# Geo3DSmart/PDANet

Hardware: AMD Instinct MI355X
Metric: scenes/sec (16384-pt ONCE, PDA-SSD forward+backward) (higher is better)
Workload: dtype f32; 1 GPU; once16k_b2_detector_fwd_bwd_adam; scenes_per_gpu=2, global_batch=2, parallelism=dp1, world_size_seen=1, cpu_affinity=GPU-local NUMA node of 0000:26:00.0: 128 CPUs, full=False, graph_tail=False, graph_head=True

## Files before the change

include/pda_train.h:

```cpp
#ifndef PDA_TRAIN_H
#define PDA_TRAIN_H
#include "pda_pointnet2.h"

#ifdef __cplusplus
extern "C" {
#endif

int pda_grad_norm(const float *g, int64_t n, float *norm_out, float *scratch1024, pda_stream_t stream);
int pda_adam_onecycle_step(float *p, const float *g, float *m, float *v, int64_t n, float lr,
                           float beta1, float beta2, float eps, float wd, int step,
                           const float *total_norm, float max_norm, pda_stream_t stream);

int64_t pda_bn_relu_scratch_bytes(int c);
int pda_bn_relu_fwd(const float *x, const float *gamma, const float *beta, float *running_mean,
                    float *running_var, float *y, float *mean_invstd, void *scratch, int64_t rows, int c,
                    float eps, float momentum, pda_stream_t stream);
int pda_bn_relu_bwd(const float *x, const float *grad_y, const float *gamma, const float *beta,
                    const float *mean_invstd, float *grad_x, float *grad_gamma, float *grad_beta,
                    void *scratch, int64_t rows, int c, pda_stream_t stream);
int pda_bn_relu_fwd_mixed(const void *x, int x_is_bf16, const float *gamma, const float *beta, float *running_mean,
                          float *running_var, void *y, int y_is_bf16, float *mean_invstd, void *scratch,
                          int64_t rows, int c, float eps, float momentum, pda_stream_t stream);
int pda_bn_relu_bwd_mixed(const void *x, int x_is_bf16, const void *grad_y, int grad_y_is_bf16, const float *gamma,
                          const float *beta, const float *mean_invstd, void *grad_x, float *grad_gamma,
                          float *grad_beta, void *scratch, int64_t rows, int c, pda_stream_t stream);
int pda_bn_relu_max_pool_fwd(const void *x, int x_is_bf16, const float *gamma, const float *beta, float *running_mean,
                             float *running_var, float *out, uint8_t *arg, float *mean_invstd, void *scratch,
                             int64_t groups, int ns, int c, float eps, float momentum, pda_stream_t stream);
int pda_bn_relu_max_pool_bwd(const void *x, int x_is_bf16, const float *grad_out, const uint8_t *arg,
                             const float *gamma, const float *beta, const float *mean_invstd, void *grad_x,
                             float *grad_gamma, float *grad_beta, void *scratch, int64_t groups, int ns, int c,
                             pda_stream_t stream);

int64_t pda_layer_norm_scratch_bytes(int d);
int pda_layer_norm_fwd(const float *x, const float *residual, const float *gamma, const float *beta,
                       float *sum_out, float *y, float *mean_rstd, int64_t rows, int d, float eps,
                       pda_stream_t stream);
int pda_layer_norm_bwd(const float *x, const float *grad_y, const float *grad_y2, const float *gamma,
                       const float *mean_rstd, float *grad_x, float *grad_gamma, float *grad_beta,
                       void *scratch, int64_t rows, int d, pda_stream_t stream);
int pda_layer_norm_fwd_mixed(const void *x, int x_is_bf16, const float *residual, const float *gamma,
                             const float *beta, float *sum_out, float *y, uint16_t *y_bf16, float *mean_rstd,
                             int64_t rows, int d, float eps, pda_stream_t stream);
int pda_layer_norm_bwd_mixed(const float *x, const float *grad_y, const void *grad_y2, int grad_y2_is_bf16,
                             const float *gamma, const float *mean_rstd, float *grad_x, uint16_t *grad_x_bf16,
                             float *grad_gamma, float *grad_beta, void *scratch, int64_t rows, int d,
                             pda_stream_t stream);

int64_t pda_linear_wgrad_scratch_bytes(int64_t tokens, int in_features, int out_features);
int pda_linear_wgrad_form(int64_t tokens, int in_features, int out_features);
int pda_linear_wgrad(const float *x, const float *grad_out, float *grad_weight, float *grad_bias,
                     void *scratch, int64_t tokens, int in_features, int out_features, pda_stream_t stream);
int pda_linear_wgrad_bn(const float *x, const float *grad_out, float *grad_weight, float *grad_bias, void *scratch,
                        int64_t tokens, int in_features, int out_features, const float *x_mean_invstd,
                        const float *x_gamma, const float *x_beta, pda_stream_t stream);

int64_t pda_gemm_split_bn_tiles(int64_t tokens);
int pda_gemm_split_bn(const float *x, const void *wf, float *y, int64_t tokens, int k, int n_out,
                      const float *in_mean_invstd, const float *in_gamma, const float *in_beta, int stats_mode,
                      double *partial, pda_stream_t stream);
int pda_gemm_split_maxpool(const float *x, const void *wf, const float *bias, float *out, int64_t tokens, int k, int n_out,
                           int ns, int relu, pda_stream_t stream);
int pda_gemm_split_gather(const float *point_rows, const float *xyz, const float *new_xyz, const int32_t *idx,
                          const float *w1, int ldw1, const float *bias1, const void *wf, const float *bias2, float *y,
                          int b, int n, int m, int ns, int k, int n_out, int relu, pda_stream_t stream);
int pda_bn_stats_fwd(const float *x, float *running_mean, float *running_var, float *mean_invstd, void *scratch,
                     int64_t rows, int c, float eps, float momentum, pda_stream_t stream);
int pda_bn_finalize_fwd(const double *partial, int nblocks, int c, int64_t count, float eps, float momentum,
                        float *mean_invstd, float *running_mean, float *running_var, pda_stream_t stream);
int pda_bn_relu_max_pool_apply(const float *x, const float *gamma, const float *beta, const float *mean_invstd,
                               float *out, uint8_t *arg, int64_t groups, int ns, int c, pda_stream_t stream);

int64_t pda_colsum_scratch_bytes(int cols);
int pda_colsum_bf16(const uint16_t *g, float *out, void *scratch, int64_t rows, int cols, pda_stream_t stream);

int pda_assemble_tokens(const float *rppe, const float *dscale, const float *feats, const int32_t *idx,
                        const float *glob, float *out, int b, int n, int m, int nsample, int c,
                        pda_stream_t stream);
int pda_assemble_tokens_grad(const float *grad_out, const float *dscale, const float *feats, const int32_t *idx,
                             float *grad_rppe, float *grad_dscale, float *grad_feats, float *grad_glob,
                             int b, int n, int m, int nsample, int c, pda_stream_t stream);

int pda_add_max_pool(const float *a, const float *b, float *out, uint8_t *arg, int64_t groups, int seq, int d,
                     pda_stream_t stream);
int pda_max_pool_scatter(const float *grad_out, const uint8_t *arg, float *grad_x, int64_t groups, int seq,
                         int d, pda_stream_t stream);
int pda_add_max_pool_bf16(const float *a, const uint16_t *b, float *out, uint8_t *arg, int64_t groups, int seq,
                          int d, pda_stream_t stream);
int pda_max_pool_scatter_bf16(const float *grad_out, const uint8_t *arg, float *grad_x, uint16_t *grad_x_bf16,
                              int64_t groups, int seq, int d, pda_stream_t stream);

int pda_bn_relu_fwd_weighted(const float *x, const float *gamma, const float *beta, float *running_mean,
                             float *running_var, float *y, float *mean_invstd, void *scratch, int64_t rows, int c,
                             float eps, float momentum, const float *row_weight, int64_t count, pda_stream_t stream);
int pda_bn_relu_bwd_weighted(const float *x, const float *grad_y, const float *gamma, const float *beta,
                             const float *mean_invstd, float *grad_x, float *grad_gamma, float *grad_beta,
                             void *scratch, int64_t rows, int c, const float *row_weight, int64_t count,
                             pda_stream_t stream);

int pda_ragged_plan(const int32_t *idx, int32_t *cnt, int32_t *off, int32_t *rowmap, float *row_weight, int64_t groups,
                    int nsample, pda_stream_t stream);
int pda_assemble_tokens_ragged(const float *rppe, const float *dscale, const float *feats, const int32_t *idx,
                               const float *glob, const int32_t *rowmap, const int32_t *off, float *out,
                               int64_t max_tokens, int b, int n, int m, int nsample, int c, int rppe_compact,
                               pda_stream_t stream);
int pda_assemble_tokens_ragged_grad(const float *grad_out, const float *dscale, const float *feats,
                                    const int32_t *idx, const int32_t *cnt, const int32_t *off, const int32_t *rowmap,
                                    float *grad_rppe, float *grad_dscale, float *grad_feats, float *grad_glob,
                                    int64_t max_tokens, int b, int n, int m, int nsample, int c, int rppe_compact,
                                    pda_stream_t stream);
int pda_add_max_pool_ragged(const float *a, const float *b, const int32_t *cnt, const int32_t *off, float *out,
                            uint8_t *arg, int64_t groups, int d, pda_stream_t stream);
int pda_max_pool_scatter_ragged(const float *grad_out, const uint8_t *arg, const int32_t *rowmap,
                                const int32_t *off, float *grad_x, int64_t max_tokens, int64_t groups, int nsample,
                                int d, pda_stream_t stream);
int pda_group_attention_ragged_fwd(const float *qkv, const int32_t *cnt, const int32_t *off, float *out, float *lse,
                                   int64_t tokens, int64_t num_groups, int seq, int heads, int head_dim,
                                   pda_stream_t stream);
int pda_group_attention_ragged_bwd(const float *qkv, const float *grad_out, const float *lse, const int32_t *cnt,
                                   const int32_t *off, float *grad_qkv, int64_t tokens, int64_t num_groups, int seq,
                                   int heads, int head_dim, pda_stream_t stream);

int pda_densitynet_param_count(void);
int64_t pda_densitynet_scratch_bytes(void);
int pda_densitynet_fwd(const float *x, const float *params, float *y, float *stats, void *scratch,
                       float *running_mean1, float *running_var1, float *running_mean2, float *running_var2,
                       float *running_mean3, float *running_var3, int64_t n, float eps, float momentum,
                       pda_stream_t stream);
int pda_densitynet_bwd(const float *x, const float *grad_y, const float *params, const float *stats,
                       float *grad_params, void *scratch, int64_t n, float eps, pda_stream_t stream);
int pda_densitynet_fwd_unique(const float *x, const float *params, float *y, float *stats, void *scratch,
                              float *running_mean1, float *running_var1, float *running_mean2, float *running_var2,
                              float *running_mean3, float *running_var3, int64_t n, const int32_t *rowmap,
                              const float *row_weight, const int32_t *n_unique, int nsample, float eps, float momentum,
                              pda_stream_t stream);
int pda_densitynet_bwd_unique(const float *x, const float *grad_y, const float *params, const float *stats,
                              float *grad_params, void *scratch, int64_t n, const int32_t *rowmap,
                              const float *row_weight, const int32_t *n_unique, int nsample, float eps,
                              pda_stream_t stream);
#define PDA_DENSITYNET_MAX_SCALES 4
typedef struct pda_densitynet_scale {
    const float *x, *grad_y, *params;
    float *y, *stats;
    void *scratch;
    float *running[6];
    float *grad_params;
    int64_t n;
    const int32_t *rowmap;
    const float *row_weight;
    const int32_t *n_unique;
    int nsample;
    float eps, momentum;
} pda_densitynet_scale_t;
int pda_densitynet_fwd_multi(const pda_densitynet_scale_t *scales, int nscales, pda_stream_t stream);
int pda_densitynet_bwd_multi(const pda_densitynet_scale_t *scales, int nscales, pda_stream_t stream);

int pda_densitynet_eval_param_count(void);
int pda_densitynet_eval(const float *x, const float *folded, float *y, int64_t n, pda_stream_t stream);

int pda_pda_geometry(const float *xyz, const float *new_xyz, const int32_t *idx, float *rppe, float *dscale,
                     int b, int n, int m, int nsample, float radius, pda_stream_t stream);

int pda_points_in_boxes(const float *boxes, const float *pts, int32_t *box_idx_of_points, int b, int t,
                        int m, pda_stream_t stream);
int pda_roiaware_pool3d_fwd(const float *rois, const float *pts, const float *pts_feature, int32_t *argmax,
                            int32_t *pts_idx_of_voxels, float *pooled_features, int boxes_num, int pts_num,
                            int channels, int max_pts_each_voxel, int out_x, int out_y, int out_z, int pool_method,
                            pda_stream_t stream);
int pda_roiaware_pool3d_bwd(const int32_t *pts_idx_of_voxels, const int32_t *argmax, const float *grad_out,
                            float *grad_in, int boxes_num, int pts_num, int channels, int max_pts_each_voxel,
                            int out_x, int out_y, int out_z, int pool_method, pda_stream_t stream);
int pda_roipoint_pool3d_fwd(const float *xyz, const float *boxes3d, const float *pts_feature, float *pooled_features,
                            int32_t *pooled_empty_flag, int batch_size, int pts_num, int boxes_num, int channels,
                            int sampled_pts_num, pda_stream_t stream);
int pda_points_in_boxes_mask(const float *boxes, const float *pts, int32_t *mask, int boxes_num, int pts_num,
                             pda_stream_t stream);
int pda_points_in_boxes_count(const float *points, int stride, const float *boxes, int32_t *counts, int pts_num,
                              int batch_size, int boxes_num, pda_stream_t stream);
int pda_assign_point_targets(const float *gt_boxes, const int32_t *in_box, const int32_t *in_ext, int64_t *labels,
                             int64_t *box_idx, float *gt_of_points, int b, int n, int t, int mode, int single_class,
                             pda_stream_t stream);
int pda_head_assign_targets(const float *points, int point_stride, int point_offset, const float *gt_boxes, const float *extra_width,
                            int64_t *labels, int64_t *box_idx, float *gt_of_points, float *box_labels, const float *mean_size,
                            int bins, int b, int n, int t, int mode, int single_class, pda_stream_t stream);
int pda_sa_gaussian_mask(const float *coords, int stride, int offset, const float *gt_of_points, const int64_t *labels,
                         float *out, int64_t points, pda_stream_t stream);

int pda_boxes_overlap_bev(const float *boxes_a, const float *boxes_b, float *ans_overlap, int num_a,
                          int num_b, pda_stream_t stream);
int pda_boxes_iou_bev(const float *boxes_a, const float *boxes_b, float *ans_iou, int num_a, int num_b,
                      pda_stream_t stream);
int64_t pda_nms_mask_words(int n);
int pda_nms_bev(const float *boxes, const int32_t *num_valid, int64_t *keep, int32_t *num_keep,
                uint64_t *mask_scratch, int b, int n, float thresh, int normal, pda_stream_t stream);

int pda_head_cls_loss(const float *preds, int row_stride, int col0, int num_class, const int64_t *labels, const float *soft,
                      int64_t n, float scale, float *out2, float *grad, pda_stream_t stream);
int pda_head_centerness(const float *centers, const float *gt, const int64_t *labels, float *out, int64_t n, pda_stream_t stream);
int pda_head_box_loss(const float *preds, const float *labels, const int64_t *cls_labels, const float *code_weights, float beta,
                      int bins, float dir_weight, float box_weight, int64_t n, float *out4, float *grad, pda_stream_t stream);
int pda_head_vote_loss(int mode, const float *origin, const float *offsets, const int64_t *key, const float *gt, int b, int boxes,
                       int num_class, float weight, int64_t n, float *out1, float *grad, pda_stream_t stream);
int pda_head_corner_loss(const float *box_preds, const float *centers, const float *cls_preds, int num_class, const float *gt,
                         const int64_t *cls_labels, const float *mean_size, int bins, float weight, int64_t n, float *out1,
                         float *grad_box, float *grad_centers, pda_stream_t stream);

int64_t pda_sa_small_train_workspace_bytes(void);
int pda_sa_small_train_supported(int c, int nsample, int c1, int c2, int c3, int64_t tokens);
int pda_sa_small_train_fwd(const float *xyz, const float *new_xyz, const float *feat_pm, const int32_t *idx,
                           const float *w1, const float *w2, const float *w3, const float *const *gamma,
                           const float *const *beta, float *const *running_mean, float *const *running_var,
                           const float *eps, const float *momentum, void *workspace, float *out, float *zmax,
                           uint8_t *arg, int b, int n, int m, int c, int nsample, int c1, int c2, int c3,
                           pda_stream_t stream);
int pda_sa_small_train_bwd(const float *xyz, const float *new_xyz, const float *feat_pm, const int32_t *idx,
                           const float *grad_out, const float *zmax, const uint8_t *arg, void *workspace, float *dz2,
                           float *dz1, float *dw1, float *dw2, float *dw3, float *const *dgamma, float *const *dbeta,
                           int b, int n, int m, int c, int nsample, int c1, int c2, int c3, pda_stream_t stream);

int64_t pda_sa_xyz_grad_scratch_bytes(int c1);
int pda_sa_point_gather(const float *point_rows, const float *xyz, const float *new_xyz, const int32_t *idx, const float *w,
                        int ldw, const float *bias, int relu, float *z, int b, int n, int m, int nsample, int c1,
                        pda_stream_t stream);
int pda_sa_xyz_grad(const float *grad_z1, const float *xyz, const float *new_xyz, const int32_t *idx, const float *w, int ldw,
                    float *dw, int lddw, float *grad_new_xyz, void *scratch, int b, int n, int m, int nsample, int c1,
                    pda_stream_t stream);

int64_t pda_input_stage_workspace_bytes(int batch, int64_t n_cap);
int pda_input_stage(const float *points, const int64_t *offsets, int64_t n_total, int batch, int c, int64_t n_cap,
                    const float *range6, int num_points, const int32_t *pick, const int32_t *perm1, const int32_t *perm2,
                    uint64_t seed, int shuffle, float *out_points, int32_t *info, void *workspace, pda_stream_t stream);
int pda_input_boxes(const float *boxes, const int64_t *box_offsets, int64_t m_total, int batch, int box_dim, int max_gt,
                    const float *range6, int min_num_corners, float *gt_boxes, int32_t *info, pda_stream_t stream);

int64_t pda_augment_workspace_bytes(int batch, int64_t n_cap, int k);
int pda_augment(const float *points, const int64_t *offsets, int64_t n_total, int batch, int c, int64_t n_cap,
                const float *boxes, const int64_t *box_offsets, int64_t m_total, const float *db_points,
                const int64_t *db_offsets, int64_t db_n_points, const float *db_boxes, const double *db_centre,
                const int32_t *db_class, int n_obj, const int32_t *cand, const int32_t *cand_group, const double *cand_dz,
                int k, const int32_t *flip, const double *angle, const float *scale, const float *remove_extra_width,
                int64_t paste_cap, float *out_points, int64_t out_cap, int64_t *out_offsets, float *out_boxes,
                int64_t out_box_cap, int64_t *out_box_offsets, int32_t *info, void *workspace, pda_stream_t stream);

int pda_augment_paste(const float *points, const int64_t *offsets, int64_t n_total, int batch, int c, int64_t n_cap,
                      const float *boxes, const int64_t *box_offsets, int64_t m_total, const float *db_points,
                      const int64_t *db_offsets, int64_t db_n_points, const float *db_boxes, const double *db_centre,
                      const int32_t *db_class, int n_obj, const int32_t *cand, const int32_t *cand_group,
                      const double *cand_dz, int k, const float *remove_extra_width, int64_t paste_cap, float *out_points,
                      int64_t out_cap, int64_t *out_offsets, float *out_boxes, int64_t out_box_cap,
                      int64_t *out_box_offsets, int32_t *info, void *workspace, pda_stream_t stream);

int64_t pda_augment_steps_workspace_bytes(int batch, int64_t n_cap, int box_slots, int n_ops);
int pda_augment_steps(const float *points, const int64_t *offsets, int64_t n_total, int batch, int c, int64_t n_cap,
                      const float *boxes, const int64_t *box_offsets, int64_t m_total, const int32_t *ops, int n_ops,
                      const double *scene_draws, const double *box_draws, int draw_cap, int box_slots,
                      const int32_t *info_in, float *out_points, int64_t out_cap, int64_t *out_offsets, float *out_boxes,
                      int64_t out_box_cap, int64_t *out_box_offsets, int32_t *info, void *workspace, pda_stream_t stream);

typedef struct pda_once_frames {
    const double *gt_boxes;
    const int32_t *gt_name;
    const int64_t *gt_offsets;
    const float *pred_boxes, *pred_score;
    const int32_t *pred_name;
    const int64_t *pred_start;
    const int32_t *pred_count;
    const int64_t *iou_start;
    int64_t n_gt_total, pred_cap, iou_cap;
    int n_frames, max_gt, max_pred;
} pda_once_frames_t;

int64_t pda_once_eval_workspace_bytes(int n_frames, int64_t n_gt_total, int n_tasks);
int pda_once_eval_iou(const pda_once_frames_t *frames, int with_heading, double *iou, int32_t *status,
                      pda_stream_t stream);
int pda_once_eval_accumulate(const pda_once_frames_t *frames, const double *iou, const uint8_t *accept, int n_classes,
                             int n_names, const double *iou_thr, int difficulty_mode, int64_t *num_valid_gt,
                             int32_t *status, void *workspace, pda_stream_t stream);
int pda_once_eval_match(const pda_once_frames_t *frames, const double *iou, const uint8_t *accept, int n_classes,
                        int n_names, const double *iou_thr, int difficulty_mode, int num_pr_points,
                        const float *sorted_scores, const int64_t *num_valid_gt, double *thresholds,
                        int64_t *n_thresholds, int64_t *counts, int32_t *status, void *workspace, pda_stream_t stream);


typedef struct pda_kitti_frames {
    const float *gt_bbox, *gt_loc;
    const double *gt_dims, *gt_ry, *gt_alpha, *gt_trunc, *gt_occ;
    const int32_t *gt_name;
    const int64_t *gt_offsets;
    const float *dt_bbox, *dt_box, *dt_alpha, *dt_score;
    const int32_t *dt_name;
    const int64_t *dt_start;
    const int32_t *dt_count;
    const int64_t *ov_start;
    const int32_t *frame_mode;
    int64_t n_gt_total, det_cap, ov_cap;
    int n_frames, max_gt, max_det;
} pda_kitti_frames_t;

int64_t pda_kitti_eval_workspace_bytes(int n_frames, int64_t n_gt_total, int64_t det_cap, int n_classes);
int pda_kitti_eval_overlaps(const pda_kitti_frames_t *frames, double *overlaps, int32_t *status, pda_stream_t stream);
int pda_kitti_eval_first_pass(const pda_kitti_frames_t *frames, const double *overlaps, int n_classes, int n_names,
                              const int8_t *gt_class, const uint8_t *dt_class, const uint8_t *dontcare,
                              const double *min_overlaps, int8_t *gt_flags, int8_t *dt_flags, int64_t *num_valid_gt,
                              int32_t *status, void *workspace, pda_stream_t stream);
int pda_kitti_eval_match(const pda_kitti_frames_t *frames, const double *overlaps, int n_classes, int n_names,
                         const int8_t *gt_class, const uint8_t *dt_class, const uint8_t *dontcare,
                         const double *min_overlaps, int compute_aos, const int8_t *gt_flags, const int8_t *dt_flags,
                         const float *sorted_scores, const int64_t *num_valid_gt, double *thresholds,
                         int64_t *n_thresholds, int64_t *counts, double *similarity, int32_t *status, void *workspace,
                         pda_stream_t stream);
int pda_kitti_eval_predictions(const float *boxes, int64_t n, int stride, int rows_per_frame, const int32_t *frame_idx,
                               const float *calib, const int32_t *image_shape, int n_frames, float *cam, float *bbox,
                               float *alpha, int32_t *status, pda_stream_t stream);

int pda_recall_record(const float *pred_boxes, const int32_t *num_pred, const float *gt_boxes, int gt_cols,
                      const float *thresh, int n_thresh, int64_t *counters, float *max_iou, int b, int k, int t,
                      pda_stream_t stream);

int pda_roi_max_iou(const float *rois, const int64_t *roi_labels, const float *gt_boxes, int gt_cols, int by_class,
                    float *max_overlaps, int32_t *gt_assignment, int b, int m, int t, pda_stream_t stream);
int pda_roi_sample_targets(const float *rois, const float *roi_scores, const int64_t *roi_labels, const float *gt_boxes,
                           int gt_cols, const float *max_overlaps, const int32_t *gt_assignment, int roi_per_image,
                           int fg_per_image, double hard_bg_ratio, double reg_fg_thresh, double cls_fg_thresh,
                           double cls_bg_thresh, double cls_bg_thresh_lo, int score_type, const int32_t *perm,
                           const double *fg_rand, const int64_t *hard_draw, const int64_t *easy_draw, uint64_t seed,
                           float *out_rois, float *gt_of_rois_src, float *gt_of_rois, float *gt_iou_of_rois,
                           float *out_roi_scores, int64_t *out_roi_labels, int64_t *reg_valid_mask, void *rcnn_cls_labels,
                           int32_t *sampled_inds, int32_t *status, int b, int m, int t, pda_stream_t stream);

int64_t pda_kitti_fov_filter_workspace_bytes(int batch, int64_t n_cap);
int pda_kitti_fov_filter(const float *points, const int64_t *offsets, int64_t n_total, int batch, int c, int64_t n_cap,
                         const float *calib, const int32_t *image_shape, float *out_points, int64_t out_cap,
                         int64_t *out_offsets, int32_t *info, void *workspace, pda_stream_t stream);
int64_t pda_gt_extract_workspace_bytes(int batch, int64_t n_cap, int64_t m_total);
int pda_gt_extract_count(const float *points, const int64_t *offsets, int64_t n_total, int batch, int c, int64_t n_cap,
                         const float *boxes, const int64_t *box_offsets, int64_t m_total, int32_t *counts, int32_t *info,
                         void *workspace, pda_stream_t stream);
int pda_gt_extract_write(const float *points, const int64_t *offsets, int64_t n_total, int batch, int c, int64_t n_cap,
                         const float *boxes, const int64_t *box_offsets, int64_t m_total, const double *centre,
                         const int64_t *obj_offsets, float *obj_points, int64_t out_cap, int32_t *info, void *workspace,
                         pda_stream_t stream);

int64_t pda_voxel_workspace_bytes(int batch, int64_t n_cap, int max_voxels, int max_points);
int pda_voxelize(const float *points, const int64_t *offsets, int64_t n_total, int batch, int c, int64_t n_cap,
                 const float *range6, const float *voxel_size3, const int32_t *grid3, int max_voxels, int max_points,
                 float *voxels, int32_t *coords, int32_t *num_points_per_voxel, int32_t *num_voxels, void *workspace,
                 pda_stream_t stream);
int pda_voxel_sample(const float *points, const int64_t *offsets, int64_t n_total, int batch, int c, int64_t n_cap,
                     const float *range6, const float *voxel_size3, const int32_t *grid3, int mask_xy, int max_voxels,
                     int max_points, int mean_vfe, int shuffle, const int32_t *perm0, const int64_t *perm0_offsets,
                     int64_t perm0_total, uint64_t seed, float *out_points, int64_t out_cap, int64_t *out_offsets,
                     int32_t *info, void *workspace, pda_stream_t stream);

int64_t pda_dyn_voxel_workspace_bytes(int64_t n, int key_bits);
int pda_dyn_voxel_index(const float *points, int64_t n, int columns, const float *range6, const float *voxel_size3,
                        const int32_t *grid3, int batch, int pillars, int32_t *counts, int32_t *point_idx, int32_t *unq_inv,
                        int32_t *unq_cnt, int32_t *voxel_coords, int32_t *seg_start, int32_t *seg_points, void *workspace,
                        pda_stream_t stream);
int pda_dyn_scatter_mean(const float *src, int columns, const int32_t *seg_start, const int32_t *seg_points,
                         const int32_t *counts, int64_t rows, float *out, pda_stream_t stream);
int pda_dyn_scatter_max_fwd(const float *x, int columns, const int32_t *seg_start, const int32_t *seg_points,
                            const int32_t *counts, int64_t rows, float *out, int32_t *arg, pda_stream_t stream);
int pda_dyn_scatter_max_bwd(const float *grad_out, const int32_t *arg, const int32_t *unq_inv, const int32_t *counts,
                            int64_t rows, int64_t vox_rows, int columns, float *grad_x, pda_stream_t stream);
int pda_dyn_pillar_features(const float *points, int64_t n, int columns, const int32_t *point_idx, const int32_t *unq_inv,
                            const int32_t *voxel_coords, const float *mean, const int32_t *counts, const float *voxel_size3,
                            const float *offset3, int absolute_xyz, int with_distance, float *out, pda_stream_t stream);

int pda_pillar_scatter_fwd(const float *features, const int32_t *coords, const int32_t *count, int64_t n, int c, int b, int ny,
                           int nx, float *out, pda_stream_t stream);
int pda_pillar_scatter_bwd(const float *grad_out, const int32_t *coords, const int32_t *count, int64_t n, int c, int b, int ny,
                           int nx, float *grad_features, pda_stream_t stream);
int pda_center_assign_targets(const float *gt_boxes, int gt_cols, int b, int m, int num_class, int n_heads,
                              const int32_t *head_of_class, const int32_t *local_of_class, const int32_t *head_classes, int h,
                              int w, int max_objs, double pcr0, double pcr1, double vs0, double vs1, double stride,
                              double gaussian_overlap, int min_radius, void *const *heatmaps, void *const *target_boxes,
                              void *const *inds, void *const *masks, pda_stream_t stream);
int64_t pda_center_focal_blocks(int64_t n);
int pda_center_focal_loss(const float *logits, const float *heatmap, int64_t n, float *grad, double *partials, float *out,
// ... 86 lines not shown
```

pdanet_amd/_lib.py:

```python
import ctypes
import os

_HERE = os.path.dirname(os.path.abspath(__file__))
LIB_PATH = os.environ.get("PDA_LIB_PATH") or os.path.join(_HERE, "libpda_pointnet2.so")
ABI_VERSION = 20


class DensityNetScale(ctypes.Structure):
    _fields_ = [("x", ctypes.c_void_p), ("grad_y", ctypes.c_void_p), ("params", ctypes.c_void_p), ("y", ctypes.c_void_p),
                ("stats", ctypes.c_void_p), ("scratch", ctypes.c_void_p), ("running", ctypes.c_void_p * 6),
                ("grad_params", ctypes.c_void_p), ("n", ctypes.c_int64), ("rowmap", ctypes.c_void_p),
                ("row_weight", ctypes.c_void_p), ("n_unique", ctypes.c_void_p), ("nsample", ctypes.c_int),
                ("eps", ctypes.c_float), ("momentum", ctypes.c_float)]


class OnceFrames(ctypes.Structure):
    _fields_ = [("gt_boxes", ctypes.c_void_p), ("gt_name", ctypes.c_void_p), ("gt_offsets", ctypes.c_void_p),
                ("pred_boxes", ctypes.c_void_p), ("pred_score", ctypes.c_void_p), ("pred_name", ctypes.c_void_p),
                ("pred_start", ctypes.c_void_p), ("pred_count", ctypes.c_void_p), ("iou_start", ctypes.c_void_p),
                ("n_gt_total", ctypes.c_int64), ("pred_cap", ctypes.c_int64), ("iou_cap", ctypes.c_int64),
                ("n_frames", ctypes.c_int), ("max_gt", ctypes.c_int), ("max_pred", ctypes.c_int)]


class KittiFrames(ctypes.Structure):
    _fields_ = [(n, ctypes.c_void_p) for n in ("gt_bbox", "gt_loc", "gt_dims", "gt_ry", "gt_alpha", "gt_trunc", "gt_occ",
                                               "gt_name", "gt_offsets", "dt_bbox", "dt_box", "dt_alpha", "dt_score",
                                               "dt_name", "dt_start", "dt_count", "ov_start", "frame_mode")] + \
               [("n_gt_total", ctypes.c_int64), ("det_cap", ctypes.c_int64), ("ov_cap", ctypes.c_int64),
                ("n_frames", ctypes.c_int), ("max_gt", ctypes.c_int), ("max_det", ctypes.c_int)]


PARAM_EPOCH = [0]
WEIGHT_EPOCH = [0]

_vp = ctypes.c_void_p
_i = ctypes.c_int
_f = ctypes.c_float

SIGNATURES = {
    "pda_furthest_point_sampling": [_vp, _vp, _vp, _i, _i, _i, _vp],
    "pda_furthest_point_sampling_with_dist": [_vp, _vp, _vp, _i, _i, _i, _vp],
    "pda_gather_points": [_vp, _vp, _vp, _i, _i, _i, _i, _vp],
    "pda_gather_points_grad": [_vp, _vp, _vp, _i, _i, _i, _i, _vp],
    "pda_ball_query": [_vp, _vp, _vp, _i, _i, _i, _f, _i, _vp],
    "pda_ball_query_dilated": [_vp, _vp, _vp, _i, _i, _i, _f, _f, _i, _vp],
    "pda_ellipsoid_query": [_vp, _vp, _vp, _i, _i, _i, _f, _f, _f, _i, _vp],
    "pda_ball_query_cells_scratch_bytes": [_i, _i],
    "pda_ball_query_cells": [_vp, _vp, ctypes.POINTER(_vp), _i, _i, _i, _i, ctypes.POINTER(_f), ctypes.POINTER(ctypes.c_int32),
                             _vp, ctypes.c_int64, _vp],
    "pda_ball_query_multi": [_vp, _vp, ctypes.POINTER(_vp), _i, _i, _i, _i,
                             ctypes.POINTER(_f), ctypes.POINTER(ctypes.c_int32), _vp],
    "pda_group_points": [_vp, _vp, _vp, _i, _i, _i, _i, _i, _vp],
    "pda_group_points_grad": [_vp, _vp, _vp, _i, _i, _i, _i, _i, _vp],
    "pda_group_rows": [_vp, _vp, _vp, _i, _i, _i, ctypes.c_int64, _vp],
    "pda_group_rows_grad": [_vp, _vp, _vp, _i, _i, _i, ctypes.c_int64, _vp],
    "pda_three_nn": [_vp, _vp, _vp, _vp, _i, _i, _i, _vp],
    "pda_three_interpolate": [_vp, _vp, _vp, _vp, _i, _i, _i, _i, _vp],
    "pda_three_interpolate_grad": [_vp, _vp, _vp, _vp, _i, _i, _i, _i, _vp],
    "pda_chamfer_forward": [_vp, _vp, _vp, _vp, _vp, _vp, _i, _i, _i, _vp],
    "pda_chamfer_backward": [_vp, _vp, _vp, _vp, _vp, _vp, _vp, _vp, _i, _i, _i, _vp],
    "pda_group_attention_fwd": [_vp, _vp, _vp, ctypes.c_int64, _i, _i, _i, _vp],
    "pda_group_attention_bwd": [_vp, _vp, _vp, _vp, ctypes.c_int64, _i, _i, _i, _vp],
    "pda_group_attention_fwd_bf16": [_vp, _vp, _vp, ctypes.c_int64, _i, _i, _i, _vp],
    "pda_group_attention_bwd_bf16": [_vp, _vp, _vp, _vp, ctypes.c_int64, _i, _i, _i, _vp],
    "pda_sa_mlp_maxpool": [_vp, _vp, _vp, _vp, _vp, _i, _i, _i, _i, _i, ctypes.POINTER(ctypes.c_int32),
                           ctypes.POINTER(_vp), ctypes.POINTER(_vp), ctypes.POINTER(_vp), _vp],
    "pda_linear_cols_packed_size": [_i, _i],
    "pda_linear_cols_pack": [_vp, _vp, _i, _i, _i, _i, _vp],
    "pda_linear_cols": [_vp, _vp, _vp, ctypes.c_int64, _i, _i, _vp],
    "pda_sa_gather_linear": [_vp, _vp, _vp, _vp, _vp, _vp, _i, _i, _i, _i, _i, _i, _vp],
    "pda_linear_split_packed_bytes": [_i, _i],
    "pda_linear_split_pack": [_vp, _vp, _i, _i, _i, _vp],
    "pda_linear_split_pack_both": [_vp, _vp, _vp, _i, _i, _vp],
    "pda_linear_split": [_vp, _vp, _vp, _vp, ctypes.c_int64, _i, _i, _i, _vp],
    "pda_gemm_split": [_vp, _vp, _vp, _vp, ctypes.c_int64, _i, _i, _i, _i, _vp],
    "pda_sa_mlp_packed_size": [_i, _i, _i],
    "pda_sa_mlp_pack_weights": [_vp, _vp, _i, _i, _i, _vp],
    "pda_grad_norm": [_vp, ctypes.c_int64, _vp, _vp, _vp],
    "pda_bn_relu_scratch_bytes": [_i],
    "pda_bn_relu_fwd": [_vp, _vp, _vp, _vp, _vp, _vp, _vp, _vp, ctypes.c_int64, _i, _f, _f, _vp],
    "pda_bn_relu_bwd": [_vp, _vp, _vp, _vp, _vp, _vp, _vp, _vp, _vp, ctypes.c_int64, _i, _vp],    "pda_bn_relu_fwd_mixed": [_vp, _i, _vp, _vp, _vp, _vp, _vp, _i, _vp, _vp, ctypes.c_int64, _i, _f, _f, _vp],
    "pda_bn_relu_bwd_mixed": [_vp, _i, _vp, _i, _vp, _vp, _vp, _vp, _vp, _vp, _vp, ctypes.c_int64, _i, _vp],
    "pda_bn_relu_max_pool_fwd": [_vp, _i, _vp, _vp, _vp, _vp, _vp, _vp, _vp, _vp, ctypes.c_int64, _i, _i, _f, _f, _vp],
    "pda_bn_relu_max_pool_bwd": [_vp, _i, _vp, _vp, _vp, _vp, _vp, _vp, _vp, _vp, _vp, ctypes.c_int64, _i, _i, _vp],

    "pda_layer_norm_scratch_bytes": [_i],
    "pda_layer_norm_fwd": [_vp, _vp, _vp, _vp, _vp, _vp, _vp, ctypes.c_int64, _i, _f, _vp],
    "pda_layer_norm_bwd": [_vp, _vp, _vp, _vp, _vp, _vp, _vp, _vp, _vp, ctypes.c_int64, _i, _vp],
    "pda_layer_norm_fwd_mixed": [_vp, _i, _vp, _vp, _vp, _vp, _vp, _vp, _vp, ctypes.c_int64, _i, _f, _vp],
    "pda_layer_norm_bwd_mixed": [_vp, _vp, _vp, _i, _vp, _vp, _vp, _vp, _vp, _vp, _vp, ctypes.c_int64, _i, _vp],
    "pda_linear_wgrad_scratch_bytes": [ctypes.c_int64, _i, _i],
    "pda_linear_wgrad_form": [ctypes.c_int64, _i, _i],
    "pda_linear_wgrad": [_vp, _vp, _vp, _vp, _vp, ctypes.c_int64, _i, _i, _vp],
    "pda_linear_wgrad_bn": [_vp, _vp, _vp, _vp, _vp, ctypes.c_int64, _i, _i, _vp, _vp, _vp, _vp],
    "pda_gemm_split_bn_tiles": [ctypes.c_int64],
    "pda_gemm_split_bn": [_vp, _vp, _vp, ctypes.c_int64, _i, _i, _vp, _vp, _vp, _i, _vp, _vp],
    "pda_gemm_split_maxpool": [_vp, _vp, _vp, _vp, ctypes.c_int64, _i, _i, _i, _i, _vp],
    "pda_gemm_split_gather": [_vp, _vp, _vp, _vp, _vp, _i, _vp, _vp, _vp, _vp, _i, _i, _i, _i, _i, _i, _i, _vp],
    "pda_bn_stats_fwd": [_vp, _vp, _vp, _vp, _vp, ctypes.c_int64, _i, _f, _f, _vp],
    "pda_bn_finalize_fwd": [_vp, _i, _i, ctypes.c_int64, _f, _f, _vp, _vp, _vp, _vp],
    "pda_bn_relu_max_pool_apply": [_vp, _vp, _vp, _vp, _vp, _vp, ctypes.c_int64, _i, _i, _vp],
    "pda_colsum_scratch_bytes": [_i],
    "pda_colsum_bf16": [_vp, _vp, _vp, ctypes.c_int64, _i, _vp],
    "pda_assemble_tokens": [_vp, _vp, _vp, _vp, _vp, _vp, _i, _i, _i, _i, _i, _vp],
    "pda_assemble_tokens_grad": [_vp, _vp, _vp, _vp, _vp, _vp, _vp, _vp, _i, _i, _i, _i, _i, _vp],
    "pda_add_max_pool": [_vp, _vp, _vp, _vp, ctypes.c_int64, _i, _i, _vp],
    "pda_max_pool_scatter": [_vp, _vp, _vp, ctypes.c_int64, _i, _i, _vp],
    "pda_add_max_pool_bf16": [_vp, _vp, _vp, _vp, ctypes.c_int64, _i, _i, _vp],
    "pda_max_pool_scatter_bf16": [_vp, _vp, _vp, _vp, ctypes.c_int64, _i, _i, _vp],
    "pda_ragged_plan": [_vp, _vp, _vp, _vp, _vp, ctypes.c_int64, _i, _vp],
    "pda_assemble_tokens_ragged": [_vp, _vp, _vp, _vp, _vp, _vp, _vp, _vp, ctypes.c_int64, _i, _i, _i, _i, _i, _i, _vp],
    "pda_assemble_tokens_ragged_grad": [_vp, _vp, _vp, _vp, _vp, _vp, _vp, _vp, _vp, _vp, _vp, ctypes.c_int64, _i, _i, _i, _i, _i, _i, _vp],
    "pda_bn_relu_fwd_weighted": [_vp, _vp, _vp, _vp, _vp, _vp, _vp, _vp, ctypes.c_int64, _i, _f, _f, _vp, ctypes.c_int64, _vp],
    "pda_bn_relu_bwd_weighted": [_vp, _vp, _vp, _vp, _vp, _vp, _vp, _vp, _vp, ctypes.c_int64, _i, _vp, ctypes.c_int64, _vp],
    "pda_add_max_pool_ragged": [_vp, _vp, _vp, _vp, _vp, _vp, ctypes.c_int64, _i, _vp],
    "pda_max_pool_scatter_ragged": [_vp, _vp, _vp, _vp, _vp, ctypes.c_int64, ctypes.c_int64, _i, _i, _vp],
    "pda_group_attention_ragged_fwd": [_vp, _vp, _vp, _vp, _vp, ctypes.c_int64, ctypes.c_int64, _i, _i, _i, _vp],
    "pda_group_attention_ragged_bwd": [_vp, _vp, _vp, _vp, _vp, _vp, ctypes.c_int64, ctypes.c_int64, _i, _i, _i, _vp],
    "pda_densitynet_param_count": [],
    "pda_densitynet_eval_param_count": [],
    "pda_densitynet_scratch_bytes": [],
    "pda_densitynet_fwd": [_vp, _vp, _vp, _vp, _vp, _vp, _vp, _vp, _vp, _vp, _vp, ctypes.c_int64, _f, _f, _vp],
    "pda_densitynet_bwd": [_vp, _vp, _vp, _vp, _vp, _vp, ctypes.c_int64, _f, _vp],
    "pda_densitynet_eval": [_vp, _vp, _vp, ctypes.c_int64, _vp],
    "pda_densitynet_fwd_multi": [_vp, _i, _vp],
    "pda_densitynet_bwd_multi": [_vp, _i, _vp],
    "pda_densitynet_fwd_unique": [_vp, _vp, _vp, _vp, _vp, _vp, _vp, _vp, _vp, _vp, _vp, ctypes.c_int64, _vp, _vp, _vp, _i, _f, _f, _vp],
    "pda_densitynet_bwd_unique": [_vp, _vp, _vp, _vp, _vp, _vp, ctypes.c_int64, _vp, _vp, _vp, _i, _f, _vp],
    "pda_pda_geometry": [_vp, _vp, _vp, _vp, _vp, _i, _i, _i, _i, _f, _vp],
    "pda_points_in_boxes": [_vp, _vp, _vp, _i, _i, _i, _vp],
    "pda_roiaware_pool3d_fwd": [_vp, _vp, _vp, _vp, _vp, _vp, _i, _i, _i, _i, _i, _i, _i, _i, _vp],
    "pda_roiaware_pool3d_bwd": [_vp, _vp, _vp, _vp, _i, _i, _i, _i, _i, _i, _i, _i, _vp],
    "pda_roipoint_pool3d_fwd": [_vp, _vp, _vp, _vp, _vp, _i, _i, _i, _i, _i, _vp],
    "pda_points_in_boxes_mask": [_vp, _vp, _vp, _i, _i, _vp],
    "pda_points_in_boxes_count": [_vp, _i, _vp, _vp, _i, _i, _i, _vp],
    "pda_assign_point_targets": [_vp, _vp, _vp, _vp, _vp, _vp, _i, _i, _i, _i, _i, _vp],
    "pda_sa_gaussian_mask": [_vp, _i, _i, _vp, _vp, _vp, ctypes.c_int64, _vp],
    "pda_head_assign_targets": [_vp, _i, _i, _vp, ctypes.POINTER(ctypes.c_float), _vp, _vp, _vp, _vp, _vp, _i, _i, _i, _i, _i, _i, _vp],
    "pda_head_cls_loss": [_vp, _i, _i, _i, _vp, _vp, ctypes.c_int64, _f, _vp, _vp, _vp],
    "pda_head_centerness": [_vp, _vp, _vp, _vp, ctypes.c_int64, _vp],
    "pda_head_box_loss": [_vp, _vp, _vp, _vp, _f, _i, _f, _f, ctypes.c_int64, _vp, _vp, _vp],
    "pda_head_vote_loss": [_i, _vp, _vp, _vp, _vp, _i, _i, _i, _f, ctypes.c_int64, _vp, _vp, _vp],
    "pda_head_corner_loss": [_vp, _vp, _vp, _i, _vp, _vp, _vp, _i, _f, ctypes.c_int64, _vp, _vp, _vp, _vp],
    "pda_boxes_overlap_bev": [_vp, _vp, _vp, _i, _i, _vp],
    "pda_boxes_iou_bev": [_vp, _vp, _vp, _i, _i, _vp],
    "pda_nms_mask_words": [_i],
    "pda_nms_bev": [_vp, _vp, _vp, _vp, _vp, _i, _i, _f, _i, _vp],
    "pda_sa_small_train_workspace_bytes": [],
    "pda_sa_small_train_supported": [_i, _i, _i, _i, _i, ctypes.c_int64],
    "pda_sa_small_train_fwd": [_vp] * 7 + [ctypes.POINTER(_vp)] * 4 + [ctypes.POINTER(_f)] * 2 + [_vp] * 4 + [_i] * 8 + [_vp],
    "pda_sa_small_train_bwd": [_vp] * 13 + [ctypes.POINTER(_vp)] * 2 + [_i] * 8 + [_vp],
    "pda_sa_xyz_grad_scratch_bytes": [_i],
    "pda_sa_point_gather": [_vp, _vp, _vp, _vp, _vp, _i, _vp, _i, _vp, _i, _i, _i, _i, _i, _vp],
    "pda_sa_xyz_grad": [_vp, _vp, _vp, _vp, _vp, _i, _vp, _i, _vp, _vp, _i, _i, _i, _i, _i, _vp],
    "pda_adam_onecycle_step": [_vp, _vp, _vp, _vp, ctypes.c_int64, _f, _f, _f, _f, _f, _i, _vp, _f, _vp],
    "pda_input_stage_workspace_bytes": [_i, ctypes.c_int64],
    "pda_input_stage": [_vp, _vp, ctypes.c_int64, _i, _i, ctypes.c_int64, ctypes.POINTER(_f), _i, _vp, _vp, _vp,
                        ctypes.c_uint64, _i, _vp, _vp, _vp, _vp],
    "pda_input_boxes": [_vp, _vp, ctypes.c_int64, _i, _i, _i, ctypes.POINTER(_f), _i, _vp, _vp, _vp],
    "pda_augment_workspace_bytes": [_i, ctypes.c_int64, _i],
    "pda_augment": [_vp, _vp, ctypes.c_int64, _i, _i, ctypes.c_int64, _vp, _vp, ctypes.c_int64, _vp, _vp, ctypes.c_int64, _vp,
                    _vp, _vp, _i, _vp, _vp, _vp, _i, _vp, _vp, _vp, ctypes.POINTER(_f), ctypes.c_int64, _vp, ctypes.c_int64,
                    _vp, _vp, ctypes.c_int64, _vp, _vp, _vp, _vp],
    "pda_augment_paste": [_vp, _vp, ctypes.c_int64, _i, _i, ctypes.c_int64, _vp, _vp, ctypes.c_int64, _vp, _vp, ctypes.c_int64, _vp,
                          _vp, _vp, _i, _vp, _vp, _vp, _i, ctypes.POINTER(_f), ctypes.c_int64, _vp, ctypes.c_int64, _vp, _vp,
                          ctypes.c_int64, _vp, _vp, _vp, _vp],
    "pda_augment_steps_workspace_bytes": [_i, ctypes.c_int64, _i, _i],
    "pda_augment_steps": [_vp, _vp, ctypes.c_int64, _i, _i, ctypes.c_int64, _vp, _vp, ctypes.c_int64,
                          ctypes.POINTER(ctypes.c_int32), _i, _vp, _vp, _i, _i, _vp, _vp, ctypes.c_int64, _vp, _vp,
                          ctypes.c_int64, _vp, _vp, _vp, _vp],
    "pda_once_eval_workspace_bytes": [_i, ctypes.c_int64, _i],
    "pda_once_eval_iou": [ctypes.POINTER(OnceFrames), _i, _vp, _vp, _vp],
    "pda_once_eval_accumulate": [ctypes.POINTER(OnceFrames), _vp, _vp, _i, _i, ctypes.POINTER(ctypes.c_double), _i, _vp, _vp,
                                 _vp, _vp],
    "pda_once_eval_match": [ctypes.POINTER(OnceFrames), _vp, _vp, _i, _i, ctypes.POINTER(ctypes.c_double), _i, _i, _vp, _vp,
                            _vp, _vp, _vp, _vp, _vp, _vp],
    "pda_kitti_eval_workspace_bytes": [_i, ctypes.c_int64, ctypes.c_int64, _i],
    "pda_kitti_eval_overlaps": [ctypes.POINTER(KittiFrames), _vp, _vp, _vp],
    "pda_kitti_eval_first_pass": [ctypes.POINTER(KittiFrames), _vp, _i, _i, _vp, _vp, _vp, ctypes.POINTER(ctypes.c_double),
                                  _vp, _vp, _vp, _vp, _vp, _vp],
    "pda_kitti_eval_match": [ctypes.POINTER(KittiFrames), _vp, _i, _i, _vp, _vp, _vp, ctypes.POINTER(ctypes.c_double), _i,
                             _vp, _vp, _vp, _vp, _vp, _vp, _vp, _vp, _vp, _vp, _vp],
    "pda_kitti_eval_predictions": [_vp, ctypes.c_int64, _i, _i, _vp, _vp, _vp, _i, _vp, _vp, _vp, _vp, _vp],
    "pda_recall_record": [_vp, _vp, _vp, _i, ctypes.POINTER(_f), _i, _vp, _vp, _i, _i, _i, _vp],
    "pda_roi_max_iou": [_vp, _vp, _vp, _i, _i, _vp, _vp, _i, _i, _i, _vp],
    "pda_roi_sample_targets": [_vp, _vp, _vp, _vp, _i, _vp, _vp, _i, _i] + [ctypes.c_double] * 5 + [_i, _vp, _vp, _vp, _vp,
                               ctypes.c_uint64] + [_vp] * 10 + [_i, _i, _i, _vp],
    "pda_kitti_fov_filter_workspace_bytes": [_i, ctypes.c_int64],
    "pda_kitti_fov_filter": [_vp, _vp, ctypes.c_int64, _i, _i, ctypes.c_int64, _vp, _vp, _vp, ctypes.c_int64, _vp, _vp, _vp, _vp],
    "pda_gt_extract_workspace_bytes": [_i, ctypes.c_int64, ctypes.c_int64],
    "pda_gt_extract_count": [_vp, _vp, ctypes.c_int64, _i, _i, ctypes.c_int64, _vp, _vp, ctypes.c_int64, _vp, _vp, _vp, _vp],
    "pda_gt_extract_write": [_vp, _vp, ctypes.c_int64, _i, _i, ctypes.c_int64, _vp, _vp, ctypes.c_int64, _vp, _vp, _vp,
                             ctypes.c_int64, _vp, _vp, _vp],
    "pda_voxel_workspace_bytes": [_i, ctypes.c_int64, _i, _i],
    "pda_voxelize": [_vp, _vp, ctypes.c_int64, _i, _i, ctypes.c_int64, ctypes.POINTER(_f), ctypes.POINTER(_f),
                     ctypes.POINTER(ctypes.c_int32), _i, _i, _vp, _vp, _vp, _vp, _vp, _vp],
    "pda_voxel_sample": [_vp, _vp, ctypes.c_int64, _i, _i, ctypes.c_int64, ctypes.POINTER(_f), ctypes.POINTER(_f),
                         ctypes.POINTER(ctypes.c_int32), _i, _i, _i, _i, _i, _vp, _vp, ctypes.c_int64, ctypes.c_uint64, _vp,
                         ctypes.c_int64, _vp, _vp, _vp, _vp],
    "pda_dyn_voxel_workspace_bytes": [ctypes.c_int64, _i],
    "pda_dyn_voxel_index": [_vp, ctypes.c_int64, _i, ctypes.POINTER(_f), ctypes.POINTER(_f), ctypes.POINTER(ctypes.c_int32),
                            _i, _i, _vp, _vp, _vp, _vp, _vp, _vp, _vp, _vp, _vp],
    "pda_dyn_scatter_mean": [_vp, _i, _vp, _vp, _vp, ctypes.c_int64, _vp, _vp],
    "pda_dyn_scatter_max_fwd": [_vp, _i, _vp, _vp, _vp, ctypes.c_int64, _vp, _vp, _vp],
    "pda_dyn_scatter_max_bwd": [_vp, _vp, _vp, _vp, ctypes.c_int64, ctypes.c_int64, _i, _vp, _vp],
    "pda_dyn_pillar_features": [_vp, ctypes.c_int64, _i, _vp, _vp, _vp, _vp, _vp, ctypes.POINTER(_f), ctypes.POINTER(_f), _i,
                                _i, _vp, _vp],
    "pda_pillar_scatter_fwd": [_vp, _vp, _vp, ctypes.c_int64, _i, _i, _i, _i, _vp, _vp],
    "pda_pillar_scatter_bwd": [_vp, _vp, _vp, ctypes.c_int64, _i, _i, _i, _i, _vp, _vp],
    "pda_center_assign_targets": [_vp, _i, _i, _i, _i, _i] + [ctypes.POINTER(ctypes.c_int32)] * 3 + [_i, _i, _i]
                                 + [ctypes.c_double] * 6 + [_i] + [ctypes.POINTER(_vp)] * 4 + [_vp],
    "pda_center_focal_blocks": [ctypes.c_int64],
    "pda_center_focal_loss": [_vp, _vp, ctypes.c_int64, _vp, _vp, _vp, _vp],
    "pda_center_scale": [_vp, _vp, _vp, _f, ctypes.c_int64, _vp, _vp],
    "pda_center_reg_loss": [ctypes.POINTER(_vp), ctypes.POINTER(ctypes.c_int32), _i, _vp, _vp, _vp, ctypes.POINTER(_f), _f, _i,
                            _i, ctypes.c_int64, _vp, _vp],
    "pda_center_reg_loss_grad": [ctypes.POINTER(_vp), ctypes.POINTER(ctypes.c_int32), _i, _vp, _vp, _vp, ctypes.POINTER(_f), _f,
                                 _i, _i, ctypes.c_int64, _vp, _vp, ctypes.POINTER(_vp), _vp],
    "pda_center_decode": [_vp] * 7 + [_i] * 5 + [ctypes.POINTER(ctypes.c_int32)] + [ctypes.c_double] * 5
                         + [ctypes.POINTER(_f), _i, ctypes.c_double, _vp, _vp, _vp, _vp],
    "pda_anchor_assign_targets": [_vp, _i, _i, _i, _vp, _i, _i, ctypes.POINTER(ctypes.c_int32), ctypes.POINTER(_f),
                                  ctypes.POINTER(_f), ctypes.POINTER(ctypes.c_int32), _vp, _vp, _vp, _vp, _vp, _vp],
    "pda_anchor_loss_blocks": [ctypes.c_int64],
    "pda_anchor_loss": [_vp] * 7 + [_i] * 4 + [ctypes.POINTER(_f)] + [ctypes.c_double] * 4 + [_vp] * 6,
    "pda_anchor_decode": [_vp, _vp, _vp, _i, _i, _i, ctypes.c_double, ctypes.c_double, _vp, _vp],
    "pda_pillar_features": [_vp, _vp, _vp, ctypes.c_int64, _i, _i, ctypes.POINTER(_f), ctypes.POINTER(_f), _i, _i, _vp, _vp],
    "pda_spconv_index_workspace_bytes": [ctypes.c_int64, ctypes.c_int64, _i],
    "pda_spconv_index_subm": [_vp, ctypes.c_int64] + [_i] * 7 + [_vp, _vp, _vp, _vp],
    "pda_spconv_index_strided": [_vp, ctypes.c_int64] + [_i] * 13 + [ctypes.c_int64, _vp, _vp, _vp, _vp, _vp, _vp],
    "pda_spconv_gemm": [_vp, _vp, _vp, _vp, _vp, ctypes.c_int64, ctypes.c_int64, _i, _i, _i, _i, _i, _vp],
    "pda_spconv_wgrad_workspace_bytes": [ctypes.c_int64, _i, _i, _i],
    "pda_spconv_wgrad": [_vp, _vp, _vp, ctypes.c_int64, ctypes.c_int64, _i, _i, _i, _vp, _vp, _vp, _vp],
    "pda_voxel_pool_scratch_doubles": [_i, _i, _i],
    "pda_voxel_pool_moments": [_vp, _vp, _vp, _vp, _vp, _i, _i, _i, _vp],
    "pda_voxel_pool_fwd": [_vp] * 9 + [_i, _i, _i, _i, _vp],
    "pda_voxel_pool_bwd": [_vp] * 10 + [_i, _i, _i, _i, _vp],
    "pda_stack_sa_scratch_doubles": [_i, _i, _i, _i],
    "pda_stack_sa_moments": [_vp] * 9 + [_i] * 5 + [_vp],
    "pda_stack_sa_fwd": [_vp] * 15 + [_i] * 6 + [_vp],
    "pda_stack_sa_apply": [_vp, _vp, _vp, _vp, _i, _i, _vp],
    "pda_stack_sa_bwd1": [_vp] * 18 + [_i] * 6 + [_vp],
    "pda_stack_sa_bwd2": [_vp] * 14 + [_i] * 5 + [_vp],
    "pda_bev_interpolate_fwd": [_vp] * 5 + [_i] * 5 + [_vp],
    "pda_bev_interpolate_bwd": [_vp] * 5 + [_i] * 5 + [_vp],
    "pda_bev_roi_grid_pool": [_vp] * 3 + [_i] * 6 + [_f] * 4 + [_vp],
    "pda_stack_ball_query": [_vp, _vp, _vp, _vp, _vp, _i, _i, _f, _i, _vp],
    "pda_stack_group_points": [_vp, _vp, _vp, _vp, _vp, _i, _i, _i, _i, _vp],
    "pda_stack_group_points_grad": [_vp, _vp, _vp, _vp, _vp, _i, _i, _i, _i, _i, _vp],
    "pda_stack_furthest_point_sampling": [_vp, _vp, _vp, _vp, _vp, _i, _vp],
    "pda_stack_three_nn": [_vp, _vp, _vp, _vp, _vp, _vp, _i, _i, _vp],
    "pda_stack_three_interpolate": [_vp, _vp, _vp, _vp, _i, _i, _vp],
    "pda_stack_three_interpolate_grad": [_vp, _vp, _vp, _vp, _i, _i, _vp],
    "pda_stack_voxel_query": [_vp, _vp, _vp, _vp, _vp, _i, _i, _i, _i, _i, _i, _i, _f, _i, _i, _i, _vp],
    "pda_stack_query_local_neighbor_idxs": [_vp, _vp, _vp, _vp, _vp, _vp, _vp, _i, _f, _i, _i, _i, _i, _vp],
    "pda_stack_three_nn_by_local_idxs": [_vp, _vp, _vp, _vp, _vp, _vp, _i, ctypes.c_int64, _i, _i, _vp],
    "pda_stack_vector_pool": [_vp, _vp, _vp, _vp, _vp, _vp, _vp, _vp, _vp, _vp, _i, _i, _i, _i, _i, _i, _i, _i, _f, _i, _i,
                              _i, _i, _i, _vp],
    "pda_stack_vector_pool_grad": [_vp, _vp, _vp, _vp, _i, _i, _i, _i, _i, _i, _vp],
}
SIZE_QUERIES = [
    "pda_nms_mask_words", "pda_ball_query_cells_scratch_bytes", "pda_bn_relu_scratch_bytes",
    "pda_layer_norm_scratch_bytes", "pda_linear_wgrad_scratch_bytes", "pda_linear_split_packed_bytes",
    "pda_colsum_scratch_bytes", "pda_gemm_split_bn_tiles", "pda_densitynet_scratch_bytes",
    "pda_sa_small_train_workspace_bytes", "pda_sa_xyz_grad_scratch_bytes", "pda_input_stage_workspace_bytes",
    "pda_augment_workspace_bytes", "pda_augment_steps_workspace_bytes", "pda_once_eval_workspace_bytes",
    "pda_kitti_eval_workspace_bytes", "pda_kitti_fov_filter_workspace_bytes", "pda_gt_extract_workspace_bytes",
    "pda_voxel_workspace_bytes", "pda_dyn_voxel_workspace_bytes", "pda_center_focal_blocks", "pda_anchor_loss_blocks",
    "pda_spconv_index_workspace_bytes", "pda_spconv_wgrad_workspace_bytes", "pda_voxel_pool_scratch_doubles",
    "pda_stack_sa_scratch_doubles"]
INFO_SYMBOLS = ["pda_abi_version", "pda_last_error", "pda_fp_contract_mode", "pda_opt_n_threads",
                "pda_fps_coop_timeouts", "pda_debug_fps_spin_limit", "pda_debug_fps_exchange_nonzero"]

_LIB = None


class PdaError(RuntimeError):
    pass


def load():
    global _LIB
    if _LIB is not None:
        return _LIB
    import torch
    if not os.path.exists(LIB_PATH):
        raise PdaError(
            "%s not found: build it with `python -m pdanet_amd.build` (hipcc, gfx950). "
            "pdanet_amd has no fallback path." % LIB_PATH)
    lib = ctypes.CDLL(LIB_PATH)
    for name, argtypes in SIGNATURES.items():
        fn = getattr(lib, name)
        fn.argtypes = argtypes
        fn.restype = _i
    for name in SIZE_QUERIES:
        getattr(lib, name).restype = ctypes.c_int64
    lib.pda_abi_version.restype = _i
    lib.pda_last_error.restype = ctypes.c_char_p
    lib.pda_fp_contract_mode.restype = _i
    lib.pda_opt_n_threads.argtypes = [_i]
    lib.pda_opt_n_threads.restype = _i
    lib.pda_fps_coop_timeouts.argtypes = [ctypes.POINTER(ctypes.c_ulonglong), _i]
    lib.pda_fps_coop_timeouts.restype = _i
    lib.pda_debug_fps_spin_limit.argtypes = [_i]
    lib.pda_debug_fps_spin_limit.restype = _i
    lib.pda_debug_fps_exchange_nonzero.argtypes = []
    lib.pda_debug_fps_exchange_nonzero.restype = ctypes.c_longlong
    if lib.pda_abi_version() != ABI_VERSION:
        raise PdaError("libpda_pointnet2.so ABI %d != binding ABI %d: rebuild"
                       % (lib.pda_abi_version(), ABI_VERSION))
    _LIB = lib
    return lib


def check(status, what):
    if status != 0:
        msg = load().pda_last_error().decode("utf-8", "replace")
        raise PdaError("%s failed with status %d: %s" % (what, status, msg))
```

pdanet_amd/csrc/bn_relu.hip:

```cpp
#include "pda_common.h"

namespace pda {

constexpr int BN_BLOCKS = 512;

struct BnShape {
    int64_t rows;
    int c, cg, rpb;
    int ns;
    const float* roww;
    int64_t count;
};

__device__ __forceinline__ float4 pooled_grad(const float* __restrict__ gout, const uint8_t* __restrict__ arg, int64_t r,
                                              int col, const BnShape& s) {
    const int64_t g = r / s.ns;
    const int t = (int)(r - g * s.ns);
    const float4 v = reinterpret_cast<const float4*>(gout)[g * s.cg + col];
    const uchar4 k = reinterpret_cast<const uchar4*>(arg)[g * s.cg + col];
    return make_float4(k.x == t ? v.x : 0.f, k.y == t ? v.y : 0.f, k.z == t ? v.z : 0.f, k.w == t ? v.w : 0.f);
}

__device__ __forceinline__ void block_reduce_cols(double (&a)[4], double (&b)[4], double* lds, int cg, int rpb, double* out_a,
                                                  double* out_b) {
// ... 175 lines not shown
}

template <typename TX>
__global__ __launch_bounds__(256) void bn_apply_pool_kernel(const TX* __restrict__ x, const float* __restrict__ mean_invstd,
                                                            const float* __restrict__ gamma, const float* __restrict__ beta,
                                                            float* __restrict__ out, uint8_t* __restrict__ arg, int64_t groups,
                                                            BnShape s) {
    const int64_t e = (int64_t)blockIdx.x * 256 + threadIdx.x;
    if (e >= groups * s.cg) return;
    const int64_t g = e / s.cg;
    const int col = (int)(e - g * s.cg);
    const float4 mu = reinterpret_cast<const float4*>(mean_invstd)[col], is = reinterpret_cast<const float4*>(mean_invstd + s.c)[col];
    const float4 gm = reinterpret_cast<const float4*>(gamma)[col], be = reinterpret_cast<const float4*>(beta)[col];
    float4 best = make_float4(-1.f, -1.f, -1.f, -1.f);
    uchar4 bi = make_uchar4(0, 0, 0, 0);
    const TX* px = x + (size_t)g * s.ns * s.c + 4 * col;
    for (int t = 0; t < s.ns; ++t) {
        const float4 v = load4(px + (size_t)t * s.c);
        const float y0 = fmaxf((v.x - mu.x) * is.x * gm.x + be.x, 0.f), y1 = fmaxf((v.y - mu.y) * is.y * gm.y + be.y, 0.f);
        const float y2 = fmaxf((v.z - mu.z) * is.z * gm.z + be.z, 0.f), y3 = fmaxf((v.w - mu.w) * is.w * gm.w + be.w, 0.f);
        if (y0 > best.x) { best.x = y0; bi.x = (uint8_t)t; }
        if (y1 > best.y) { best.y = y1; bi.y = (uint8_t)t; }
        if (y2 > best.z) { best.z = y2; bi.z = (uint8_t)t; }
        if (y3 > best.w) { best.w = y3; bi.w = (uint8_t)t; }
    }
    reinterpret_cast<float4*>(out)[e] = best;
    reinterpret_cast<uchar4*>(arg)[e] = bi;
}

static int bn_shape(int64_t rows, int c, BnShape& s, const char* what) {
    PDA_REQUIRE(rows >= 1, "%s: rows = %lld", what, (long long)rows);
    PDA_REQUIRE(c >= 4 && c <= 1024 && (c & (c - 1)) == 0, "%s: C = %d is not a power of two in [4, 1024]", what, c);
    s.rows = rows; s.c = c; s.cg = c / 4; s.rpb = 256 / s.cg; s.ns = 1;
    s.roww = nullptr; s.count = rows;
    return PDA_OK;
}

static int bn_grid(const BnShape& s) {
    const int64_t steps = divup64(s.rows, s.rpb);
    return (int)(steps < BN_BLOCKS ? steps : BN_BLOCKS);
}

}

PDA_API int64_t pda_bn_relu_scratch_bytes(int c) {
    const int64_t cc = c > 0 ? c : 0;
    return (int64_t)pda::BN_BLOCKS * 2 * cc * (int64_t)sizeof(double) + 2 * cc * (int64_t)sizeof(float);
}

namespace pda {

template <typename T> static bool bn_aligned(const T* p) { return ((uintptr_t)p & (4 * sizeof(T) - 1)) == 0; }

template <typename TX, typename TY>
static int launch_bn_relu_fwd(const TX* x, const float* gamma, const float* beta, float* running_mean, float* running_var, TY* y,
                              float* mean_invstd, void* scratch, int64_t rows, int c, float eps, float momentum, hipStream_t st,
                              const char* what, const float* roww = nullptr, int64_t count = 0) {
    BnShape s;
    if (int rc = bn_shape(rows, c, s, what)) return rc;
    if (roww) { PDA_REQUIRE(count >= rows, "%s: count = %lld < rows", what, (long long)count); s.roww = roww; s.count = count; }
    PDA_REQUIRE(x && gamma && beta && y && mean_invstd && scratch, "%s: null pointer", what);
    PDA_REQUIRE((running_mean == nullptr) == (running_var == nullptr), "%s: running_mean/var must come together", what);
    PDA_REQUIRE(bn_aligned(x) && bn_aligned(y) && (((uintptr_t)gamma | (uintptr_t)beta | (uintptr_t)mean_invstd) & 15) == 0,
                "%s: pointers must be 16-byte aligned (8 for bf16 tensors)", what);
    const int grid = bn_grid(s);
    hipLaunchKernelGGL((bn_reduce_kernel<false, TX, float>), dim3(grid), dim3(256), 0, st, x, (const float*)nullptr, (const float*)nullptr,
                       (const float*)nullptr, (const float*)nullptr, (double*)scratch, s);
    hipLaunchKernelGGL(bn_finalize_fwd_kernel, dim3(divup(c, 32)), dim3(512), 0, st, (const double*)scratch, grid, c, s.count, eps, momentum,
                       mean_invstd, running_mean, running_var);
    hipLaunchKernelGGL((bn_apply_kernel<false, TX, float, TY>), dim3(grid), dim3(256), 0, st, x, (const float*)nullptr, mean_invstd, gamma, beta,
                       (const float*)nullptr, y, s);
    return check_launch(what);
}

template <typename TX, typename TD>
static int launch_bn_relu_bwd(const TX* x, const TD* grad_y, const float* gamma, const float* beta, const float* mean_invstd, TX* grad_x,
                              float* grad_gamma, float* grad_beta, void* scratch, int64_t rows, int c, hipStream_t st, const char* what,
                              const float* roww = nullptr, int64_t count = 0) {
    BnShape s;
    if (int rc = bn_shape(rows, c, s, what)) return rc;
    if (roww) { PDA_REQUIRE(count >= rows, "%s: count = %lld < rows", what, (long long)count); s.roww = roww; s.count = count; }
    PDA_REQUIRE(x && grad_y && gamma && beta && mean_invstd && grad_x && grad_gamma && grad_beta && scratch, "%s: null pointer", what);
    PDA_REQUIRE(bn_aligned(x) && bn_aligned(grad_y) && bn_aligned(grad_x) && (((uintptr_t)gamma | (uintptr_t)beta | (uintptr_t)mean_invstd) & 15) == 0,
                "%s: pointers must be 16-byte aligned (8 for bf16 tensors)", what);
    const int grid = bn_grid(s);
    float* sums = reinterpret_cast<float*>(reinterpret_cast<double*>(scratch) + (size_t)BN_BLOCKS * 2 * c);
    hipLaunchKernelGGL((bn_reduce_kernel<true, TX, TD>), dim3(grid), dim3(256), 0, st, x, grad_y, mean_invstd, gamma, beta, (double*)scratch, s);
    hipLaunchKernelGGL(bn_finalize_bwd_kernel, dim3(divup(c, 32)), dim3(512), 0, st, (const double*)scratch, grid, c, s.count, grad_gamma, grad_beta,
                       sums);
    hipLaunchKernelGGL((bn_apply_kernel<true, TX, TD, TX>), dim3(grid), dim3(256), 0, st, x, grad_y, mean_invstd, gamma, beta, sums, grad_x, s);
    return check_launch(what);
}

template <typename TX>
static int launch_bn_relu_pool_fwd(const TX* x, const float* gamma, const float* beta, float* running_mean, float* running_var, float* out,
                                   uint8_t* arg, float* mean_invstd, void* scratch, int64_t groups, int ns, int c, float eps,
                                   float momentum, hipStream_t st, const char* what) {
    PDA_REQUIRE(groups >= 1 && ns >= 1 && ns <= 255, "%s: groups=%lld ns=%d (1..255)", what, (long long)groups, ns);
    BnShape s;
    if (int rc = bn_shape(groups * ns, c, s, what)) return rc;
    s.ns = ns;
    PDA_REQUIRE(x && gamma && beta && out && arg && mean_invstd && scratch, "%s: null pointer", what);
    PDA_REQUIRE((running_mean == nullptr) == (running_var == nullptr), "%s: running_mean/var must come together", what);
    PDA_REQUIRE(bn_aligned(x) && (((uintptr_t)out | (uintptr_t)gamma | (uintptr_t)beta | (uintptr_t)mean_invstd) & 15) == 0 &&
                    ((uintptr_t)arg & 3) == 0, "%s: alignment", what);
    const int grid = bn_grid(s);
    hipLaunchKernelGGL((bn_reduce_kernel<false, TX, float>), dim3(grid), dim3(256), 0, st, x, (const float*)nullptr, (const float*)nullptr,
                       (const float*)nullptr, (const float*)nullptr, (double*)scratch, s, (const uint8_t*)nullptr);
    hipLaunchKernelGGL(bn_finalize_fwd_kernel, dim3(divup(c, 32)), dim3(512), 0, st, (const double*)scratch, grid, c, s.rows, eps, momentum,
                       mean_invstd, running_mean, running_var);
    hipLaunchKernelGGL(bn_apply_pool_kernel<TX>, dim3((unsigned)divup64(groups * s.cg, 256)), dim3(256), 0, st, x, mean_invstd, gamma, beta, out,
                       arg, groups, s);
    return check_launch(what);
}

template <typename TX>
static int launch_bn_relu_pool_bwd(const TX* x, const float* grad_out, const uint8_t* arg, const float* gamma, const float* beta,
                                   const float* mean_invstd, TX* grad_x, float* grad_gamma, float* grad_beta, void* scratch, int64_t groups,
                                   int ns, int c, hipStream_t st, const char* what) {
    PDA_REQUIRE(groups >= 1 && ns >= 1 && ns <= 255, "%s: groups=%lld ns=%d (1..255)", what, (long long)groups, ns);
    BnShape s;
    if (int rc = bn_shape(groups * ns, c, s, what)) return rc;
    s.ns = ns;
    PDA_REQUIRE(x && grad_out && arg && gamma && beta && mean_invstd && grad_x && grad_gamma && grad_beta && scratch, "%s: null pointer", what);
    PDA_REQUIRE(bn_aligned(x) && bn_aligned(grad_x) && (((uintptr_t)grad_out | (uintptr_t)gamma | (uintptr_t)beta | (uintptr_t)mean_invstd) & 15) == 0 &&
                    ((uintptr_t)arg & 3) == 0, "%s: alignment", what);
    const int grid = bn_grid(s);
    float* sums = reinterpret_cast<float*>(reinterpret_cast<double*>(scratch) + (size_t)BN_BLOCKS * 2 * c);
    hipLaunchKernelGGL((bn_reduce_kernel<true, TX, float, true>), dim3(grid), dim3(256), 0, st, x, grad_out, mean_invstd, gamma, beta,
                       (double*)scratch, s, arg);
    hipLaunchKernelGGL(bn_finalize_bwd_kernel, dim3(divup(c, 32)), dim3(512), 0, st, (const double*)scratch, grid, c, s.rows, grad_gamma, grad_beta,
                       sums);
    hipLaunchKernelGGL((bn_apply_kernel<true, TX, float, TX, true>), dim3(grid), dim3(256), 0, st, x, grad_out, mean_invstd, gamma, beta, sums,
                       grad_x, s, arg);
    return check_launch(what);
}

}

PDA_API int pda_bn_relu_fwd(const float* x, const float* gamma, const float* beta, float* running_mean, float* running_var,
                            float* y, float* mean_invstd, void* scratch, int64_t rows, int c, float eps, float momentum,
                            pda_stream_t stream) {
    return pda::launch_bn_relu_fwd<float, float>(x, gamma, beta, running_mean, running_var, y, mean_invstd, scratch, rows, c, eps, momentum,
                                                 (hipStream_t)stream, "pda_bn_relu_fwd");
}

PDA_API int pda_bn_relu_bwd(const float* x, const float* grad_y, const float* gamma, const float* beta, const float* mean_invstd,
                            float* grad_x, float* grad_gamma, float* grad_beta, void* scratch, int64_t rows, int c,
                            pda_stream_t stream) {
    return pda::launch_bn_relu_bwd<float, float>(x, grad_y, gamma, beta, mean_invstd, grad_x, grad_gamma, grad_beta, scratch, rows, c,
                                                 (hipStream_t)stream, "pda_bn_relu_bwd");
}

PDA_API int pda_bn_relu_fwd_weighted(const float* x, const float* gamma, const float* beta, float* running_mean, float* running_var,
                                     float* y, float* mean_invstd, void* scratch, int64_t rows, int c, float eps, float momentum,
                                     const float* row_weight, int64_t count, pda_stream_t stream) {
    PDA_REQUIRE(row_weight != nullptr, "pda_bn_relu_fwd_weighted: null pointer");
    return pda::launch_bn_relu_fwd<float, float>(x, gamma, beta, running_mean, running_var, y, mean_invstd, scratch, rows, c, eps, momentum,
                                                 (hipStream_t)stream, "pda_bn_relu_fwd_weighted", row_weight, count);
}

PDA_API int pda_bn_relu_bwd_weighted(const float* x, const float* grad_y, const float* gamma, const float* beta, const float* mean_invstd,
                                     float* grad_x, float* grad_gamma, float* grad_beta, void* scratch, int64_t rows, int c,
                                     const float* row_weight, int64_t count, pda_stream_t stream) {
    PDA_REQUIRE(row_weight != nullptr, "pda_bn_relu_bwd_weighted: null pointer");
    return pda::launch_bn_relu_bwd<float, float>(x, grad_y, gamma, beta, mean_invstd, grad_x, grad_gamma, grad_beta, scratch, rows, c,
                                                 (hipStream_t)stream, "pda_bn_relu_bwd_weighted", row_weight, count);
}

PDA_API int pda_bn_relu_fwd_mixed(const void* x, int x_is_bf16, const float* gamma, const float* beta, float* running_mean,
                                  float* running_var, void* y, int y_is_bf16, float* mean_invstd, void* scratch, int64_t rows, int c,
                                  float eps, float momentum, pda_stream_t stream) {
    using pda::bf16_t;
    hipStream_t st = (hipStream_t)stream;
    const char* what = "pda_bn_relu_fwd_mixed";
#define PDA_BN_FWD(TX, TY) pda::launch_bn_relu_fwd<TX, TY>((const TX*)x, gamma, beta, running_mean, running_var, (TY*)y, mean_invstd, scratch, rows, c, eps, momentum, st, what)
    if (x_is_bf16) return y_is_bf16 ? PDA_BN_FWD(bf16_t, bf16_t) : PDA_BN_FWD(bf16_t, float);
    return y_is_bf16 ? PDA_BN_FWD(float, bf16_t) : PDA_BN_FWD(float, float);
#undef PDA_BN_FWD
}

PDA_API int pda_bn_relu_bwd_mixed(const void* x, int x_is_bf16, const void* grad_y, int grad_y_is_bf16, const float* gamma,
                                  const float* beta, const float* mean_invstd, void* grad_x, float* grad_gamma, float* grad_beta,
                                  void* scratch, int64_t rows, int c, pda_stream_t stream) {
    using pda::bf16_t;
    hipStream_t st = (hipStream_t)stream;
    const char* what = "pda_bn_relu_bwd_mixed";
#define PDA_BN_BWD(TX, TD) pda::launch_bn_relu_bwd<TX, TD>((const TX*)x, (const TD*)grad_y, gamma, beta, mean_invstd, (TX*)grad_x, grad_gamma, grad_beta, scratch, rows, c, st, what)
    if (x_is_bf16) return grad_y_is_bf16 ? PDA_BN_BWD(bf16_t, bf16_t) : PDA_BN_BWD(bf16_t, float);
    return grad_y_is_bf16 ? PDA_BN_BWD(float, bf16_t) : PDA_BN_BWD(float, float);
#undef PDA_BN_BWD
}

PDA_API int pda_bn_relu_max_pool_fwd(const void* x, int x_is_bf16, const float* gamma, const float* beta, float* running_mean,
                                     float* running_var, float* out, uint8_t* arg, float* mean_invstd, void* scratch, int64_t groups,
                                     int ns, int c, float eps, float momentum, pda_stream_t stream) {
    const char* what = "pda_bn_relu_max_pool_fwd";
    if (x_is_bf16)
        return pda::launch_bn_relu_pool_fwd<pda::bf16_t>((const pda::bf16_t*)x, gamma, beta, running_mean, running_var, out, arg, mean_invstd,
                                                         scratch, groups, ns, c, eps, momentum, (hipStream_t)stream, what);
    return pda::launch_bn_relu_pool_fwd<float>((const float*)x, gamma, beta, running_mean, running_var, out, arg, mean_invstd, scratch, groups,
                                               ns, c, eps, momentum, (hipStream_t)stream, what);
}

PDA_API int pda_bn_relu_max_pool_bwd(const void* x, int x_is_bf16, const float* grad_out, const uint8_t* arg, const float* gamma,
                                     const float* beta, const float* mean_invstd, void* grad_x, float* grad_gamma, float* grad_beta,
                                     void* scratch, int64_t groups, int ns, int c, pda_stream_t stream) {
    const char* what = "pda_bn_relu_max_pool_bwd";
    if (x_is_bf16)
        return pda::launch_bn_relu_pool_bwd<pda::bf16_t>((const pda::bf16_t*)x, grad_out, arg, gamma, beta, mean_invstd, (pda::bf16_t*)grad_x,
                                                         grad_gamma, grad_beta, scratch, groups, ns, c, (hipStream_t)stream, what);
    return pda::launch_bn_relu_pool_bwd<float>((const float*)x, grad_out, arg, gamma, beta, mean_invstd, (float*)grad_x, grad_gamma, grad_beta,
                                               scratch, groups, ns, c, (hipStream_t)stream, what);
}

PDA_API int pda_bn_stats_fwd(const float* x, float* running_mean, float* running_var, float* mean_invstd, void* scratch, int64_t rows, int c,
                             float eps, float momentum, pda_stream_t stream) {
    const char* what = "pda_bn_stats_fwd";
    pda::BnShape s;
    if (int rc = pda::bn_shape(rows, c, s, what)) return rc;
    PDA_REQUIRE(x && mean_invstd && scratch && pda::bn_aligned(x) && ((uintptr_t)mean_invstd & 15) == 0, "%s: null or misaligned pointer", what);
    PDA_REQUIRE((running_mean == nullptr) == (running_var == nullptr), "%s: running_mean/var must come together", what);
    const int grid = pda::bn_grid(s);
    hipStream_t st = (hipStream_t)stream;
    hipLaunchKernelGGL((pda::bn_reduce_kernel<false, float, float>), dim3(grid), dim3(256), 0, st, x, (const float*)nullptr, (const float*)nullptr,
                       (const float*)nullptr, (const float*)nullptr, (double*)scratch, s);
    hipLaunchKernelGGL(pda::bn_finalize_fwd_kernel, dim3(pda::divup(c, 32)), dim3(512), 0, st, (const double*)scratch, grid, c, s.count, eps, momentum,
                       mean_invstd, running_mean, running_var);
    return pda::check_launch(what);
}

PDA_API int pda_bn_finalize_fwd(const double* partial, int nblocks, int c, int64_t count, float eps, float momentum, float* mean_invstd,
                                float* running_mean, float* running_var, pda_stream_t stream) {
    PDA_REQUIRE(partial && mean_invstd && nblocks >= 1 && c >= 1 && count >= 1, "pda_bn_finalize_fwd: bad argument");
    PDA_REQUIRE((running_mean == nullptr) == (running_var == nullptr), "pda_bn_finalize_fwd: running_mean/var must come together");
    hipLaunchKernelGGL(pda::bn_finalize_fwd_kernel, dim3(pda::divup(c, 32)), dim3(512), 0, (hipStream_t)stream, partial, nblocks, c, count, eps,
                       momentum, mean_invstd, running_mean, running_var);
    return pda::check_launch("pda_bn_finalize_fwd");
}

PDA_API int pda_bn_relu_max_pool_apply(const float* x, const float* gamma, const float* beta, const float* mean_invstd, float* out, uint8_t* arg,
                                       int64_t groups, int ns, int c, pda_stream_t stream) {
    const char* what = "pda_bn_relu_max_pool_apply";
    PDA_REQUIRE(groups >= 1 && ns >= 1 && ns <= 255, "%s: groups=%lld ns=%d (1..255)", what, (long long)groups, ns);
    pda::BnShape s;
    if (int rc = pda::bn_shape(groups * ns, c, s, what)) return rc;
    s.ns = ns;
    PDA_REQUIRE(x && gamma && beta && out && arg && mean_invstd, "%s: null pointer", what);
    PDA_REQUIRE(pda::bn_aligned(x) && (((uintptr_t)out | (uintptr_t)gamma | (uintptr_t)beta | (uintptr_t)mean_invstd) & 15) == 0 &&
                    ((uintptr_t)arg & 3) == 0, "%s: alignment", what);
    hipLaunchKernelGGL(pda::bn_apply_pool_kernel<float>, dim3((unsigned)pda::divup64(groups * s.cg, 256)), dim3(256), 0, (hipStream_t)stream, x,
                       mean_invstd, gamma, beta, out, arg, groups, s);
    return pda::check_launch(what);
}
```

pdanet_amd/csrc/sa_xyz_grad.hip:

```cpp
#include "pda_common.h"

namespace pda {

constexpr int XG_BLOCKS = 512;
constexpr int XG_THREADS = 256;
constexpr int XG_MAXC = 4;

template <int CPT>
__global__ __launch_bounds__(XG_THREADS) void sa_xyz_grad_kernel(const float* __restrict__ g, const float* __restrict__ xyz,
                                                                 const float* __restrict__ new_xyz, const int32_t* __restrict__ idx,
                                                                 const float* __restrict__ w, int ldw, float* __restrict__ partial,
                                                                 float* __restrict__ grad_new, int n, int m, int ns, int c1, int64_t groups) {
    __shared__ float red[XG_THREADS / 64][3];
    const int tid = threadIdx.x;
    float accw[CPT][3], wx[CPT][3];
#pragma unroll
    for (int q = 0; q < CPT; ++q) {
        const int o = tid + q * XG_THREADS;
#pragma unroll
        for (int d = 0; d < 3; ++d) { accw[q][d] = 0.f; wx[q][d] = o < c1 ? w[(size_t)o * ldw + d] : 0.f; }
    }
    for (int64_t grp = blockIdx.x; grp < groups; grp += gridDim.x) {
        const int bs = (int)(grp / m);
        const float* ct = new_xyz + grp * 3;
        const float cx = ct[0], cy = ct[1], cz = ct[2];
        const float* pts = xyz + (size_t)bs * n * 3;
        const int32_t* ids = idx + grp * ns;
        const float* grow = g + grp * ns * (int64_t)c1;
        float gs[CPT];
#pragma unroll
        for (int q = 0; q < CPT; ++q) gs[q] = 0.f;
        for (int s0 = 0; s0 < ns; s0 += 8) {
            float gv[8][CPT], dx[8], dy[8], dz[8];
#pragma unroll
            for (int u = 0; u < 8; ++u) {
                const int s = s0 + u < ns ? s0 + u : ns - 1;
                const float* pt = pts + (size_t)ids[s] * 3;
                dx[u] = pt[0] - cx; dy[u] = pt[1] - cy; dz[u] = pt[2] - cz;
#pragma unroll
                for (int q = 0; q < CPT; ++q) {
                    const int o = tid + q * XG_THREADS;
                    gv[u][q] = (s0 + u < ns && o < c1) ? grow[(int64_t)s * c1 + o] : 0.f;
                }
            }
#pragma unroll
            for (int u = 0; u < 8; ++u)
#pragma unroll
                for (int q = 0; q < CPT; ++q) {
                    accw[q][0] = __builtin_fmaf(gv[u][q], dx[u], accw[q][0]);
                    accw[q][1] = __builtin_fmaf(gv[u][q], dy[u], accw[q][1]);
                    accw[q][2] = __builtin_fmaf(gv[u][q], dz[u], accw[q][2]);
                    gs[q] += gv[u][q];
                }
        }
        if (grad_new) {
            float v[3] = {0.f, 0.f, 0.f};
#pragma unroll
            for (int q = 0; q < CPT; ++q)
#pragma unroll
                for (int d = 0; d < 3; ++d) v[d] = __builtin_fmaf(gs[q], wx[q][d], v[d]);
#pragma unroll
            for (int d = 0; d < 3; ++d) {
#pragma unroll
                for (int o = 32; o >= 1; o >>= 1) v[d] += __shfl_xor(v[d], o);
            }
            __syncthreads();
            if (lane_id() == 0) { red[wave_id()][0] = v[0]; red[wave_id()][1] = v[1]; red[wave_id()][2] = v[2]; }
            __syncthreads();
            if (tid < 3) grad_new[grp * 3 + tid] = -((red[0][tid] + red[1][tid]) + (red[2][tid] + red[3][tid]));
        }
    }
#pragma unroll
    for (int q = 0; q < CPT; ++q) {
        const int o = tid + q * XG_THREADS;
        if (o < c1) {
            float* p = partial + ((size_t)blockIdx.x * c1 + o) * 3;
            p[0] = accw[q][0]; p[1] = accw[q][1]; p[2] = accw[q][2];
        }
    }
}

__global__ __launch_bounds__(256) void sa_xyz_grad_reduce_kernel(const float* __restrict__ partial, int nblocks, int c1, float* __restrict__ dw, int lddw) {
    __shared__ double red[16][16];
    const int el = threadIdx.x & 15, part = threadIdx.x >> 4;
    const int e = blockIdx.x * 16 + el;
    const bool ok = e < c1 * 3;
    double a = 0.0;
    if (ok)
        for (int k = part; k < nblocks; k += 16) a += (double)partial[(size_t)k * c1 * 3 + e];
    red[part][el] = a;
    __syncthreads();
    if (part == 0 && ok) {
        double t = 0.0;
#pragma unroll
        for (int q = 0; q < 16; ++q) t += red[q][el];
        dw[(size_t)(e / 3) * lddw + e % 3] = (float)t;
    }
}

__global__ __launch_bounds__(256) void sa_point_gather_kernel(const float* __restrict__ prow, const float* __restrict__ xyz,
                                                              const float* __restrict__ new_xyz, const int32_t* __restrict__ idx,
                                                              const float* __restrict__ w, int ldw, const float* __restrict__ bias,
                                                              int relu, float* __restrict__ z, int n, int m, int ns, int c1,
                                                              int64_t tokens) {
    const int cq = c1 >> 2;
    const int q = threadIdx.x % cq;
    float wx[4], wy[4], wz[4];
#pragma unroll
    for (int k = 0; k < 4; ++k) {
        const float* wr = w + (size_t)(4 * q + k) * ldw;
        wx[k] = wr[0]; wy[k] = wr[1]; wz[k] = wr[2];
    }
    float bq[4] = {0.f, 0.f, 0.f, 0.f};
    if (bias) { const float4 b4 = *reinterpret_cast<const float4*>(bias + 4 * q); bq[0] = b4.x; bq[1] = b4.y; bq[2] = b4.z; bq[3] = b4.w; }
    const int tpb = 256 / cq;
    for (int64_t tok = (int64_t)blockIdx.x * tpb + threadIdx.x / cq; tok < tokens; tok += (int64_t)gridDim.x * tpb) {
        const int64_t grp = tok / ns;
        const int bs = (int)(grp / m);
        const int id = idx[tok];
        const float* pt = xyz + ((size_t)bs * n + id) * 3;
        const float* ct = new_xyz + grp * 3;
        const float dx = pt[0] - ct[0], dy = pt[1] - ct[1], dz = pt[2] - ct[2];
        const float4 p4 = *reinterpret_cast<const float4*>(prow + ((size_t)bs * n + id) * c1 + 4 * q);
        const float pv[4] = {p4.x, p4.y, p4.z, p4.w};
        float o[4];
#pragma unroll
        for (int k = 0; k < 4; ++k) {
            o[k] = __builtin_fmaf(wz[k], dz, __builtin_fmaf(wy[k], dy, __builtin_fmaf(wx[k], dx, pv[k]))) + bq[k];
            o[k] = relu ? fmaxf(o[k], 0.f) : o[k];
        }
        *reinterpret_cast<float4*>(z + tok * c1 + 4 * q) = make_float4(o[0], o[1], o[2], o[3]);
    }
}

}

PDA_API int pda_sa_point_gather(const float* point_rows, const float* xyz, const float* new_xyz, const int32_t* idx, const float* w, int ldw,
                                const float* bias, int relu, float* z, int b, int n, int m, int ns, int c1, pda_stream_t stream) {
    using namespace pda;
    PDA_REQUIRE(b >= 0 && n >= 1 && m >= 0 && ns >= 1 && c1 >= 4 && (c1 & 3) == 0 && ldw >= 3, "pda_sa_point_gather: bad size");
    const int64_t tokens = (int64_t)b * m * ns;
    if (tokens == 0) return PDA_OK;
    PDA_REQUIRE(point_rows && xyz && new_xyz && idx && w && z && (((uintptr_t)point_rows | (uintptr_t)z | (uintptr_t)bias) & 15) == 0,
                "pda_sa_point_gather: null or misaligned pointer");
    if (256 % (c1 >> 2) != 0) {
        set_error("pda_sa_point_gather: c1 = %d (c1 / 4 must divide 256)", c1);
        return PDA_ERR_UNSUPPORTED;
    }
    const int64_t total = tokens * (c1 >> 2);
    const int blocks = (int)(divup64(total, 256) < 8192 ? divup64(total, 256) : 8192);
    hipLaunchKernelGGL(sa_point_gather_kernel, dim3(blocks), dim3(256), 0, (hipStream_t)stream, point_rows, xyz, new_xyz, idx, w, ldw, bias, relu, z,
                       n, m, ns, c1, tokens);
    return check_launch("pda_sa_point_gather");
}

PDA_API int64_t pda_sa_xyz_grad_scratch_bytes(int c1) { return c1 > 0 ? (int64_t)pda::XG_BLOCKS * c1 * 3 * sizeof(float) : 0; }

PDA_API int pda_sa_xyz_grad(const float* grad_z1, const float* xyz, const float* new_xyz, const int32_t* idx, const float* w, int ldw,
                            float* dw, int lddw, float* grad_new_xyz, void* scratch, int b, int n, int m, int ns, int c1,
                            pda_stream_t stream) {
    using namespace pda;
    PDA_REQUIRE(b >= 0 && n >= 1 && m >= 0 && ns >= 1 && c1 >= 1 && ldw >= 3 && lddw >= 3, "pda_sa_xyz_grad: bad size");
    const int64_t groups = (int64_t)b * m;
    if (groups == 0) return PDA_OK;
    PDA_REQUIRE(grad_z1 && xyz && new_xyz && idx && w && dw && scratch, "pda_sa_xyz_grad: null pointer");
    if (c1 > XG_THREADS * XG_MAXC) {
        set_error("pda_sa_xyz_grad: c1 = %d > %d", c1, XG_THREADS * XG_MAXC);
        return PDA_ERR_UNSUPPORTED;
    }
    const hipStream_t s = (hipStream_t)stream;
    const int blocks = (int)(groups < XG_BLOCKS ? groups : XG_BLOCKS);
    float* partial = (float*)scratch;
    const int cpt = divup(c1, XG_THREADS);
#define PDA_XG(CPT) hipLaunchKernelGGL((sa_xyz_grad_kernel<CPT>), dim3(blocks), dim3(XG_THREADS), 0, s, grad_z1, xyz, new_xyz, idx, w, ldw, \
                                       partial, grad_new_xyz, n, m, ns, c1, groups)
    if (cpt == 1) PDA_XG(1); else if (cpt == 2) PDA_XG(2); else PDA_XG(4);
#undef PDA_XG
    hipLaunchKernelGGL(sa_xyz_grad_reduce_kernel, dim3(divup(c1 * 3, 16)), dim3(256), 0, s, (const float*)partial, blocks, c1, dw, lddw);
    return check_launch("pda_sa_xyz_grad");
}
```

pdanet_amd/pointnet2_batch_cuda.py:

```python
import ctypes

import functools

import torch

from . import _lib
from . import param_cache


def _chk(t, name, dtype):
    if not isinstance(t, torch.Tensor):
        raise TypeError("%s must be a torch.Tensor" % name)
    if not t.is_cuda:
        raise RuntimeError("%s must be a CUDA(HIP) tensor -- there is no CPU path" % name)
    if not t.is_contiguous():
        raise RuntimeError("%s must be contiguous" % name)
    if t.dtype != dtype:
        raise RuntimeError("%s must be %s, got %s" % (name, dtype, t.dtype))
    return t.data_ptr()


def _numel_ok(t, n, name):
    if t.numel() < n:
        raise RuntimeError("%s has %d elements, the sizes passed need %d" % (name, t.numel(), n))
# ... 113 lines not shown
    _numel_ok(idx, b * npoints * nsample, "idx"); _numel_ok(grad_points, b * c * n, "grad_points")
    _call("pda_group_points_grad", grad_out, _chk(grad_out, "grad_out", F32), _chk(idx, "idx", I32),
          _chk(grad_points, "grad_points", F32), b, c, n, npoints, nsample)
    return 1


def group_rows(b, n, c, num_idx, rows, idx, out):
    _numel_ok(rows, b * n * c, "rows"); _numel_ok(idx, b * num_idx, "idx"); _numel_ok(out, b * num_idx * c, "out")
    _call("pda_group_rows", rows, _chk(rows, "rows", F32), _chk(idx, "idx", I32), _chk(out, "out", F32),
          b, n, c, num_idx)
    return 1


def group_rows_grad(b, n, c, num_idx, grad_out, idx, grad_rows):
    _numel_ok(grad_out, b * num_idx * c, "grad_out"); _numel_ok(idx, b * num_idx, "idx")
    _numel_ok(grad_rows, b * n * c, "grad_rows")
    _call("pda_group_rows_grad", grad_out, _chk(grad_out, "grad_out", F32), _chk(idx, "idx", I32),
          _chk(grad_rows, "grad_rows", F32), b, n, c, num_idx)
    return 1


def gather_points_wrapper(b, c, n, npoints, points, idx, out):
    _numel_ok(points, b * c * n, "points"); _numel_ok(idx, b * npoints, "idx")
    _numel_ok(out, b * c * npoints, "out")
    _call("pda_gather_points", points, _chk(points, "points", F32), _chk(idx, "idx", I32),
          _chk(out, "out", F32), b, c, n, npoints)
    return 1


def gather_points_grad_wrapper(b, c, n, npoints, grad_out, idx, grad_points):
    _numel_ok(grad_out, b * c * npoints, "grad_out"); _numel_ok(idx, b * npoints, "idx")
    _numel_ok(grad_points, b * c * n, "grad_points")
    _call("pda_gather_points_grad", grad_out, _chk(grad_out, "grad_out", F32), _chk(idx, "idx", I32),
          _chk(grad_points, "grad_points", F32), b, c, n, npoints)
    return 1


def farthest_point_sampling_wrapper(b, n, m, xyz, temp, idx):
    _numel_ok(xyz, b * n * 3, "xyz"); _numel_ok(temp, b * n, "temp"); _numel_ok(idx, b * m, "idx")
    _call("pda_furthest_point_sampling", xyz, _chk(xyz, "xyz", F32), _chk(temp, "temp", F32),
          _chk(idx, "idx", I32), b, n, m)
    return 1


def furthest_point_sampling_with_dist_wrapper(b, n, m, dist, temp, idx):
    _numel_ok(dist, b * n * n, "dist"); _numel_ok(temp, b * n, "temp"); _numel_ok(idx, b * m, "idx")
    _call("pda_furthest_point_sampling_with_dist", dist, _chk(dist, "dist", F32),
          _chk(temp, "temp", F32), _chk(idx, "idx", I32), b, n, m)
    return 2


def three_nn_wrapper(b, n, m, unknown, known, dist2, idx):
    _numel_ok(unknown, b * n * 3, "unknown"); _numel_ok(known, b * m * 3, "known")
    _numel_ok(dist2, b * n * 3, "dist2"); _numel_ok(idx, b * n * 3, "idx")
    _call("pda_three_nn", unknown, _chk(unknown, "unknown", F32), _chk(known, "known", F32),
          _chk(dist2, "dist2", F32), _chk(idx, "idx", I32), b, n, m)


def three_interpolate_wrapper(b, c, m, n, points, idx, weight, out):
    _numel_ok(points, b * c * m, "points"); _numel_ok(idx, b * n * 3, "idx")
    _numel_ok(weight, b * n * 3, "weight"); _numel_ok(out, b * c * n, "out")
    _call("pda_three_interpolate", points, _chk(points, "points", F32), _chk(idx, "idx", I32),
          _chk(weight, "weight", F32), _chk(out, "out", F32), b, c, m, n)


def three_interpolate_grad_wrapper(b, c, n, m, grad_out, idx, weight, grad_points):
    _numel_ok(grad_out, b * c * n, "grad_out"); _numel_ok(idx, b * n * 3, "idx")
    _numel_ok(weight, b * n * 3, "weight"); _numel_ok(grad_points, b * c * m, "grad_points")
    _call("pda_three_interpolate_grad", grad_out, _chk(grad_out, "grad_out", F32),
          _chk(idx, "idx", I32), _chk(weight, "weight", F32),
          _chk(grad_points, "grad_points", F32), b, c, n, m)


def chamfer_forward(xyz1, xyz2, dist1, dist2, idx1, idx2):
    b, n, _ = xyz1.shape
    m = xyz2.shape[1]
    _numel_ok(dist1, b * n, "dist1"); _numel_ok(dist2, b * m, "dist2")
    _numel_ok(idx1, b * n, "idx1"); _numel_ok(idx2, b * m, "idx2")
    _call("pda_chamfer_forward", xyz1, _chk(xyz1, "xyz1", F32), _chk(xyz2, "xyz2", F32), _chk(dist1, "dist1", F32),
          _chk(dist2, "dist2", F32), _chk(idx1, "idx1", I32), _chk(idx2, "idx2", I32), b, n, m)
    return 1


def chamfer_backward(xyz1, xyz2, gradxyz1, gradxyz2, graddist1, graddist2, idx1, idx2):
    b, n, _ = xyz1.shape
    m = xyz2.shape[1]
    _call("pda_chamfer_backward", xyz1, _chk(xyz1, "xyz1", F32), _chk(xyz2, "xyz2", F32),
          _chk(gradxyz1, "gradxyz1", F32), _chk(gradxyz2, "gradxyz2", F32), _chk(graddist1, "graddist1", F32),
          _chk(graddist2, "graddist2", F32), _chk(idx1, "idx1", I32), _chk(idx2, "idx2", I32), b, n, m)
    return 1


def group_attention_fwd(qkv, out, lse, num_groups, seq, heads, head_dim):
    _numel_ok(qkv, num_groups * seq * 3 * heads * head_dim, "qkv")
    _numel_ok(out, num_groups * seq * heads * head_dim, "out"); _numel_ok(lse, num_groups * heads * seq, "lse")
    io, sfx = (torch.bfloat16, "_bf16") if qkv.dtype == torch.bfloat16 else (F32, "")
    _call("pda_group_attention_fwd" + sfx, qkv, _chk(qkv, "qkv", io), _chk(out, "out", io), _chk(lse, "lse", F32),
          num_groups, seq, heads, head_dim)
    return 1


def group_attention_bwd(qkv, grad_out, lse, grad_qkv, num_groups, seq, heads, head_dim):
    _numel_ok(qkv, num_groups * seq * 3 * heads * head_dim, "qkv"); _numel_ok(grad_qkv, qkv.numel(), "grad_qkv")
    _numel_ok(grad_out, num_groups * seq * heads * head_dim, "grad_out"); _numel_ok(lse, num_groups * heads * seq, "lse")
    io, sfx = (torch.bfloat16, "_bf16") if qkv.dtype == torch.bfloat16 else (F32, "")
    _call("pda_group_attention_bwd" + sfx, qkv, _chk(qkv, "qkv", io), _chk(grad_out, "grad_out", io),
          _chk(lse, "lse", F32), _chk(grad_qkv, "grad_qkv", io), num_groups, seq, heads, head_dim)
    return 1


@functools.lru_cache(maxsize=None)
def bn_relu_scratch_bytes(c):
    return int(_lib.load().pda_bn_relu_scratch_bytes(int(c)))


def _io(t, name):
    if t.dtype == torch.bfloat16:
        return _chk(t, name, torch.bfloat16), 1
    return _chk(t, name, F32), 0


def _buffers_written(running):
    if running is not None:
        param_cache.buffers_written()


def bn_relu_fwd(x, gamma, beta, running_mean, running_var, y, mean_invstd, scratch, rows, c, eps, momentum):
    _numel_ok(x, rows * c, "x"); _numel_ok(y, rows * c, "y"); _numel_ok(mean_invstd, 2 * c, "mean_invstd")
    rm = None if running_mean is None else _chk(running_mean, "running_mean", F32)
    rv = None if running_var is None else _chk(running_var, "running_var", F32)
    _buffers_written(rm)
    if x.dtype == F32 and y.dtype == F32:
        _call("pda_bn_relu_fwd", x, _chk(x, "x", F32), _chk(gamma, "gamma", F32), _chk(beta, "beta", F32), rm, rv,
              _chk(y, "y", F32), _chk(mean_invstd, "mean_invstd", F32), _chk(scratch, "scratch", torch.uint8), rows, c,
              float(eps), float(momentum))
        return 1
    (xp, xb), (yp, yb) = _io(x, "x"), _io(y, "y")
    _call("pda_bn_relu_fwd_mixed", x, xp, xb, _chk(gamma, "gamma", F32), _chk(beta, "beta", F32), rm, rv, yp, yb,
          _chk(mean_invstd, "mean_invstd", F32), _chk(scratch, "scratch", torch.uint8), rows, c, float(eps), float(momentum))
    return 1


def bn_relu_bwd(x, grad_y, gamma, beta, mean_invstd, grad_x, grad_gamma, grad_beta, scratch, rows, c):
    _numel_ok(x, rows * c, "x"); _numel_ok(grad_y, rows * c, "grad_y"); _numel_ok(grad_x, rows * c, "grad_x")
    if x.dtype == F32 and grad_y.dtype == F32:
        _call("pda_bn_relu_bwd", x, _chk(x, "x", F32), _chk(grad_y, "grad_y", F32), _chk(gamma, "gamma", F32),
              _chk(beta, "beta", F32), _chk(mean_invstd, "mean_invstd", F32), _chk(grad_x, "grad_x", F32),
              _chk(grad_gamma, "grad_gamma", F32), _chk(grad_beta, "grad_beta", F32), _chk(scratch, "scratch", torch.uint8), rows, c)
        return 1
    (xp, xb), (gp, gb) = _io(x, "x"), _io(grad_y, "grad_y")
    _call("pda_bn_relu_bwd_mixed", x, xp, xb, gp, gb, _chk(gamma, "gamma", F32), _chk(beta, "beta", F32),
          _chk(mean_invstd, "mean_invstd", F32), _chk(grad_x, "grad_x", x.dtype), _chk(grad_gamma, "grad_gamma", F32),
          _chk(grad_beta, "grad_beta", F32), _chk(scratch, "scratch", torch.uint8), rows, c)
    return 1


def bn_relu_max_pool_fwd(x, gamma, beta, running_mean, running_var, out, arg, mean_invstd, scratch, groups, ns, c, eps, momentum):
    _numel_ok(x, groups * ns * c, "x"); _numel_ok(out, groups * c, "out"); _numel_ok(arg, groups * c, "arg"); _numel_ok(mean_invstd, 2 * c, "mean_invstd")
    rm = None if running_mean is None else _chk(running_mean, "running_mean", F32)
    rv = None if running_var is None else _chk(running_var, "running_var", F32)
    _buffers_written(rm)
    xp, xb = _io(x, "x")
    _call("pda_bn_relu_max_pool_fwd", x, xp, xb, _chk(gamma, "gamma", F32), _chk(beta, "beta", F32), rm, rv, _chk(out, "out", F32),
          _chk(arg, "arg", torch.uint8), _chk(mean_invstd, "mean_invstd", F32), _chk(scratch, "scratch", torch.uint8), groups, ns, c,
          float(eps), float(momentum))
    return 1


def bn_relu_max_pool_bwd(x, grad_out, arg, gamma, beta, mean_invstd, grad_x, grad_gamma, grad_beta, scratch, groups, ns, c):
    _numel_ok(x, groups * ns * c, "x"); _numel_ok(grad_out, groups * c, "grad_out"); _numel_ok(arg, groups * c, "arg")
    _numel_ok(grad_x, groups * ns * c, "grad_x")
    xp, xb = _io(x, "x")
    _call("pda_bn_relu_max_pool_bwd", x, xp, xb, _chk(grad_out, "grad_out", F32), _chk(arg, "arg", torch.uint8), _chk(gamma, "gamma", F32),
          _chk(beta, "beta", F32), _chk(mean_invstd, "mean_invstd", F32), _chk(grad_x, "grad_x", x.dtype), _chk(grad_gamma, "grad_gamma", F32),
          _chk(grad_beta, "grad_beta", F32), _chk(scratch, "scratch", torch.uint8), groups, ns, c)
    return 1


@functools.lru_cache(maxsize=None)
def layer_norm_scratch_bytes(d):
    return int(_lib.load().pda_layer_norm_scratch_bytes(int(d)))


BF16 = torch.bfloat16


def layer_norm_fwd(x, residual, gamma, beta, sum_out, y, mean_rstd, rows, d, eps, y_bf16=None):
    _numel_ok(x, rows * d, "x"); _numel_ok(mean_rstd, rows * 2, "mean_rstd")
    res = None if residual is None else _chk(residual, "residual", F32)
    so = None if sum_out is None else _chk(sum_out, "sum_out", F32)
    if x.dtype == F32 and y_bf16 is None:
        _numel_ok(y, rows * d, "y")
        _call("pda_layer_norm_fwd", x, _chk(x, "x", F32), res, _chk(gamma, "gamma", F32), _chk(beta, "beta", F32), so,
              _chk(y, "y", F32), _chk(mean_rstd, "mean_rstd", F32), rows, d, float(eps))
        return 1
    yp = yb = None
    if y is not None:
        _numel_ok(y, rows * d, "y"); yp = _chk(y, "y", F32)
    if y_bf16 is not None:
        _numel_ok(y_bf16, rows * d, "y_bf16"); yb = _chk(y_bf16, "y_bf16", BF16)
    _call("pda_layer_norm_fwd_mixed", x, _chk(x, "x", x.dtype if x.dtype == BF16 else F32), int(x.dtype == BF16), res,
          _chk(gamma, "gamma", F32), _chk(beta, "beta", F32), so, yp, yb, _chk(mean_rstd, "mean_rstd", F32), rows, d, float(eps))
    return 1


def layer_norm_bwd(x, grad_y, gamma, mean_rstd, grad_x, grad_gamma, grad_beta, scratch, rows, d, grad_y2=None, grad_x_bf16=None):
    _numel_ok(x, rows * d, "x"); _numel_ok(grad_y, rows * d, "grad_y"); _numel_ok(grad_x, rows * d, "grad_x")
    g2 = None
    if grad_y2 is not None:
        _numel_ok(grad_y2, rows * d, "grad_y2")
        g2 = _chk(grad_y2, "grad_y2", BF16 if grad_y2.dtype == BF16 else F32)
    if grad_x_bf16 is not None or (grad_y2 is not None and grad_y2.dtype == BF16):
        gxb = None
        if grad_x_bf16 is not None:
            _numel_ok(grad_x_bf16, rows * d, "grad_x_bf16"); gxb = _chk(grad_x_bf16, "grad_x_bf16", BF16)
        _call("pda_layer_norm_bwd_mixed", x, _chk(x, "x", F32), _chk(grad_y, "grad_y", F32), g2,
              int(grad_y2 is not None and grad_y2.dtype == BF16), _chk(gamma, "gamma", F32), _chk(mean_rstd, "mean_rstd", F32),
              _chk(grad_x, "grad_x", F32), gxb, _chk(grad_gamma, "grad_gamma", F32), _chk(grad_beta, "grad_beta", F32),
              _chk(scratch, "scratch", torch.uint8), rows, d)
        return 1
    _call("pda_layer_norm_bwd", x, _chk(x, "x", F32), _chk(grad_y, "grad_y", F32), g2, _chk(gamma, "gamma", F32),
          _chk(mean_rstd, "mean_rstd", F32), _chk(grad_x, "grad_x", F32), _chk(grad_gamma, "grad_gamma", F32),
          _chk(grad_beta, "grad_beta", F32), _chk(scratch, "scratch", torch.uint8), rows, d)
    return 1


_WGRAD_SCRATCH_BYTES = {}


def _wgrad_scratch_bytes(tokens, in_features, out_features):
    key = (tokens, in_features, out_features)
    nbytes = _WGRAD_SCRATCH_BYTES.get(key)
    if nbytes is None:
        if len(_WGRAD_SCRATCH_BYTES) >= 4096:
            _WGRAD_SCRATCH_BYTES.clear()
        nbytes = _WGRAD_SCRATCH_BYTES[key] = int(_lib.load().pda_linear_wgrad_scratch_bytes(tokens, in_features, out_features))
    return nbytes


@functools.lru_cache(maxsize=None)
def _split_packed_bytes(n_out, k):
    return int(_lib.load().pda_linear_split_packed_bytes(n_out, k))


@functools.lru_cache(maxsize=None)
def _cols_packed_size(n_out, k):
    return int(_lib.load().pda_linear_cols_packed_size(n_out, k))


def linear_wgrad(x, grad_out, grad_weight, grad_bias, tokens, in_features, out_features):
    _numel_ok(x, tokens * in_features, "x"); _numel_ok(grad_out, tokens * out_features, "grad_out")
    _numel_ok(grad_weight, in_features * out_features, "grad_weight")
    nbytes = _wgrad_scratch_bytes(tokens, in_features, out_features)
    scratch = torch.empty((nbytes,), dtype=torch.uint8, device=x.device)
    gb = None if grad_bias is None else _chk(grad_bias, "grad_bias", F32)
    _call("pda_linear_wgrad", x, _chk(x, "x", F32), _chk(grad_out, "grad_out", F32), _chk(grad_weight, "grad_weight", F32),
          gb, _chk(scratch, "scratch", torch.uint8), tokens, in_features, out_features)
    return 1


def linear_wgrad_bn(x, grad_out, grad_weight, tokens, in_features, out_features, x_mean_invstd, x_gamma, x_beta):
    _numel_ok(x, tokens * in_features, "x"); _numel_ok(grad_out, tokens * out_features, "grad_out")
    _numel_ok(grad_weight, in_features * out_features, "grad_weight"); _numel_ok(x_mean_invstd, 2 * in_features, "x_mean_invstd")
    _numel_ok(x_gamma, in_features, "x_gamma"); _numel_ok(x_beta, in_features, "x_beta")
    nbytes = _wgrad_scratch_bytes(tokens, in_features, out_features)
    scratch = torch.empty((nbytes,), dtype=torch.uint8, device=x.device)
    _call("pda_linear_wgrad_bn", x, _chk(x, "x", F32), _chk(grad_out, "grad_out", F32), _chk(grad_weight, "grad_weight", F32), None,
          _chk(scratch, "scratch", torch.uint8), tokens, in_features, out_features, _chk(x_mean_invstd, "x_mean_invstd", F32),
          _chk(x_gamma, "x_gamma", F32), _chk(x_beta, "x_beta", F32))
    return 1


def gemm_split_bn_tiles(tokens):
    return (int(tokens) + 255) // 256


def gemm_split_bn(x, wf, y, tokens, k, n_out, in_bn=None, stats_mode=0, partial=None):
    _numel_ok(x, tokens * k, "x"); _numel_ok(y, tokens * n_out, "y")
    _numel_ok(wf, _split_packed_bytes(int(n_out), int(k)), "wf")
    ib = (None, None, None)
    if in_bn is not None:
        _numel_ok(in_bn[0], 2 * k, "in_mean_invstd"); _numel_ok(in_bn[1], k, "in_gamma"); _numel_ok(in_bn[2], k, "in_beta")
        ib = tuple(_chk(t, "in_bn", F32) for t in in_bn)
    if stats_mode:
        _numel_ok(partial, gemm_split_bn_tiles(tokens) * 2 * n_out, "partial")
    _call("pda_gemm_split_bn", x, _chk(x, "x", F32), _chk(wf, "wf", torch.uint8), _chk(y, "y", F32), tokens, k, n_out, ib[0], ib[1], ib[2],
          int(stats_mode), None if partial is None else _chk(partial, "partial", torch.float64))
    return 1


def gemm_split_maxpool(x, wf, bias, out, tokens, k, n_out, ns, relu=True):
    _numel_ok(x, tokens * k, "x"); _numel_ok(out, (tokens // ns) * n_out, "out")
    _numel_ok(wf, _split_packed_bytes(int(n_out), int(k)), "wf")
    if bias is not None:
        _numel_ok(bias, n_out, "bias")
    _call("pda_gemm_split_maxpool", x, _chk(x, "x", F32), _chk(wf, "wf", torch.uint8), None if bias is None else _chk(bias, "bias", F32),
          _chk(out, "out", F32), tokens, k, n_out, ns, 1 if relu else 0)
    return 1


def gemm_split_gather(point_rows, xyz, new_xyz, idx, w1, bias1, wf, bias2, y, b, n, m, ns, k, n_out, relu=True):
    t = b * m * ns
    _numel_ok(point_rows, b * n * k, "point_rows"); _numel_ok(xyz, b * n * 3, "xyz"); _numel_ok(new_xyz, b * m * 3, "new_xyz")
    _numel_ok(idx, t, "idx"); _numel_ok(y, t * n_out, "y"); _numel_ok(wf, _split_packed_bytes(int(n_out), int(k)), "wf")
    if w1.dim() != 2 or w1.shape[0] != k or w1.shape[1] < 3:
        raise RuntimeError("w1 must be (k, 3 + c)")
# ... 230 lines not shown
          _chk(rowmap, "rowmap", I32), _chk(off, "off", I32), _chk(grad_x, "grad_x", F32), tokens, groups, nsample, d)
    return 1


def group_attention_ragged_fwd(qkv, cnt, off, out, lse, tokens, num_groups, seq, heads, head_dim):
    _numel_ok(qkv, tokens * 3 * heads * head_dim, "qkv"); _numel_ok(out, tokens * heads * head_dim, "out")
    _numel_ok(lse, num_groups * heads * seq, "lse"); _numel_ok(cnt, num_groups, "cnt"); _numel_ok(off, num_groups + 1, "off")
    _call("pda_group_attention_ragged_fwd", qkv, _chk(qkv, "qkv", F32), _chk(cnt, "cnt", I32), _chk(off, "off", I32),
          _chk(out, "out", F32), _chk(lse, "lse", F32), tokens, num_groups, seq, heads, head_dim)
    return 1


def group_attention_ragged_bwd(qkv, grad_out, lse, cnt, off, grad_qkv, tokens, num_groups, seq, heads, head_dim):
    _numel_ok(qkv, tokens * 3 * heads * head_dim, "qkv"); _numel_ok(grad_qkv, tokens * 3 * heads * head_dim, "grad_qkv")
    _numel_ok(grad_out, tokens * heads * head_dim, "grad_out"); _numel_ok(lse, num_groups * heads * seq, "lse")
    _call("pda_group_attention_ragged_bwd", qkv, _chk(qkv, "qkv", F32), _chk(grad_out, "grad_out", F32), _chk(lse, "lse", F32),
          _chk(cnt, "cnt", I32), _chk(off, "off", I32), _chk(grad_qkv, "grad_qkv", F32), tokens, num_groups, seq, heads, head_dim)
    return 1


def linear_cols_pack(w, n_out, k, transposed_source=False, gather_order=False):
    lib = _lib.load()
    wf = torch.empty((_cols_packed_size(int(n_out), int(k)),), dtype=F32, device=w.device)
    _numel_ok(w, n_out * k, "w")
    _call("pda_linear_cols_pack", w, _chk(w, "w", F32), _chk(wf, "wf", F32), n_out, k, 1 if transposed_source else 0,
          1 if gather_order else 0)
    return wf


def linear_cols(x, wf, y, tokens, k, n_out):
    _numel_ok(x, tokens * k, "x"); _numel_ok(y, tokens * n_out, "y")
    _numel_ok(wf, _cols_packed_size(int(n_out), int(k)), "wf")
    _call("pda_linear_cols", x, _chk(x, "x", F32), _chk(wf, "wf", F32), _chk(y, "y", F32), tokens, k, n_out)
    return 1


def linear_split_pack(w, n_out, k, transposed_source=False):
    lib = _lib.load()
    wf = torch.empty((_split_packed_bytes(int(n_out), int(k)),), dtype=torch.uint8, device=w.device)
    _numel_ok(w, n_out * k, "w")
    _call("pda_linear_split_pack", w, _chk(w, "w", F32), _chk(wf, "wf", torch.uint8), n_out, k, 1 if transposed_source else 0)
    return wf


def linear_split_pack_both(w, n_out, k):
    wf = torch.empty((_split_packed_bytes(int(n_out), int(k)),), dtype=torch.uint8, device=w.device)
    wft = torch.empty((_split_packed_bytes(int(k), int(n_out)),), dtype=torch.uint8, device=w.device)
    _numel_ok(w, n_out * k, "w")
    _call("pda_linear_split_pack_both", w, _chk(w, "w", F32), _chk(wf, "wf", torch.uint8), _chk(wft, "wft", torch.uint8), n_out, k)
    return wf, wft


def linear_split(x, wf, bias, y, tokens, k, n_out, relu=False):
    _numel_ok(x, tokens * k, "x"); _numel_ok(y, tokens * n_out, "y")
    _numel_ok(wf, _split_packed_bytes(int(n_out), int(k)), "wf")
    if bias is not None:
        _numel_ok(bias, n_out, "bias")
    _call("pda_linear_split", x, _chk(x, "x", F32), _chk(wf, "wf", torch.uint8), None if bias is None else _chk(bias, "bias", F32),
          _chk(y, "y", F32), tokens, k, n_out, 1 if relu else 0)
    return 1


def gemm_split(x, wf, bias, y, tokens, k, n_out, relu=False, accumulate=False):
    _numel_ok(x, tokens * k, "x"); _numel_ok(y, tokens * n_out, "y")
    _numel_ok(wf, _split_packed_bytes(int(n_out), int(k)), "wf")
    if bias is not None:
        _numel_ok(bias, n_out, "bias")
    _call("pda_gemm_split", x, _chk(x, "x", F32), _chk(wf, "wf", torch.uint8), None if bias is None else _chk(bias, "bias", F32),
          _chk(y, "y", F32), tokens, k, n_out, 1 if relu else 0, 1 if accumulate else 0)
    return 1


def sa_gather_linear(xyz, new_xyz, feats_pm, idx, wf, y, b, n, m, c, nsample, n_out):
    _numel_ok(xyz, b * n * 3, "xyz"); _numel_ok(new_xyz, b * m * 3, "new_xyz"); _numel_ok(feats_pm, b * n * c, "feats_pm")
    _numel_ok(idx, b * m * nsample, "idx"); _numel_ok(y, b * m * nsample * n_out, "y")
    _numel_ok(wf, _cols_packed_size(int(n_out), 3 + int(c)), "wf")
    _call("pda_sa_gather_linear", xyz, _chk(xyz, "xyz", F32), _chk(new_xyz, "new_xyz", F32), _chk(feats_pm, "feats_pm", F32),
          _chk(idx, "idx", I32), _chk(wf, "wf", F32), _chk(y, "y", F32), b, n, m, c, nsample, n_out)
    return 1


@functools.lru_cache(maxsize=None)
def sa_small_train_workspace_bytes():
    return int(_lib.load().pda_sa_small_train_workspace_bytes())


@functools.lru_cache(maxsize=None)
def sa_small_train_supported(c, ns, c1, c2, c3, tokens):
    return bool(_lib.load().pda_sa_small_train_supported(int(c), int(ns), int(c1), int(c2), int(c3), int(tokens)))


def sa_small_train_fwd(xyz, new_xyz, feat_pm, idx, weights, gammas, betas, running_means, running_vars, eps, momentum,
                       workspace, out, zmax, arg, b, n, m, c, ns):
    c1, c2, c3 = (int(w.shape[0]) for w in weights)
    tokens = b * m * ns
    _numel_ok(xyz, b * n * 3, "xyz"); _numel_ok(new_xyz, b * m * 3, "new_xyz"); _numel_ok(idx, tokens, "idx")
    _numel_ok(out, b * m * c3, "out"); _numel_ok(zmax, b * m * c3, "zmax"); _numel_ok(arg, b * m * c3, "arg")
    _numel_ok(workspace, sa_small_train_workspace_bytes(), "workspace")
    assert weights[0].shape[1] == 3 + c and weights[1].shape[1] == c1 and weights[2].shape[1] == c2
    if feat_pm is not None:
        _numel_ok(feat_pm, b * n * c, "feat_pm")
    rm = [None if t is None else _chk(t, "running_mean", F32) for t in running_means]
    rv = [None if t is None else _chk(t, "running_var", F32) for t in running_vars]
    _buffers_written(rm[0] or rm[1] or rm[2])
    _call("pda_sa_small_train_fwd", xyz, _chk(xyz, "xyz", F32), _chk(new_xyz, "new_xyz", F32),
          None if feat_pm is None else _chk(feat_pm, "feat_pm", F32), _chk(idx, "idx", I32),
          _chk(weights[0], "w1", F32), _chk(weights[1], "w2", F32), _chk(weights[2], "w3", F32),
          _ptr_array([_chk(t, "gamma", F32) for t in gammas]), _ptr_array([_chk(t, "beta", F32) for t in betas]),
          _ptr_array(rm), _ptr_array(rv), (ctypes.c_float * 3)(*[float(e) for e in eps]),
          (ctypes.c_float * 3)(*[float(x) for x in momentum]), _chk(workspace, "workspace", torch.uint8),
          _chk(out, "out", F32), _chk(zmax, "zmax", F32), _chk(arg, "arg", torch.uint8), b, n, m, c, ns, c1, c2, c3)
    return 1


def sa_small_train_bwd(xyz, new_xyz, feat_pm, idx, grad_out, zmax, arg, workspace, dz2, dz1, dws, dgammas, dbetas, b, n, m, c, ns):
    c1, c2, c3 = (int(w.shape[0]) for w in dws)
    tokens = b * m * ns
    _numel_ok(grad_out, b * m * c3, "grad_out"); _numel_ok(dz2, tokens * c2, "dz2"); _numel_ok(dz1, tokens * c1, "dz1")
    _numel_ok(workspace, sa_small_train_workspace_bytes(), "workspace")
    _call("pda_sa_small_train_bwd", xyz, _chk(xyz, "xyz", F32), _chk(new_xyz, "new_xyz", F32),
          None if feat_pm is None else _chk(feat_pm, "feat_pm", F32), _chk(idx, "idx", I32), _chk(grad_out, "grad_out", F32),
          _chk(zmax, "zmax", F32), _chk(arg, "arg", torch.uint8), _chk(workspace, "workspace", torch.uint8),
          _chk(dz2, "dz2", F32), _chk(dz1, "dz1", F32), _chk(dws[0], "dw1", F32), _chk(dws[1], "dw2", F32), _chk(dws[2], "dw3", F32),
          _ptr_array([_chk(t, "dgamma", F32) for t in dgammas]), _ptr_array([_chk(t, "dbeta", F32) for t in dbetas]),
          b, n, m, c, ns, c1, c2, c3)
    return 1


@functools.lru_cache(maxsize=None)
def sa_xyz_grad_scratch_bytes(c1):
    return int(_lib.load().pda_sa_xyz_grad_scratch_bytes(int(c1)))


def sa_xyz_grad(grad_z1, xyz, new_xyz, idx, w, dw, grad_new_xyz, b, n, m, ns, c1):
    _numel_ok(grad_z1, b * m * ns * c1, "grad_z1"); _numel_ok(idx, b * m * ns, "idx")
    _numel_ok(xyz, b * n * 3, "xyz"); _numel_ok(new_xyz, b * m * 3, "new_xyz")
    assert w.shape[0] == c1 and dw.shape == w.shape and w.shape[1] >= 3
    scratch = torch.empty((sa_xyz_grad_scratch_bytes(c1),), dtype=torch.uint8, device=xyz.device)
    _call("pda_sa_xyz_grad", xyz, _chk(grad_z1, "grad_z1", F32), _chk(xyz, "xyz", F32), _chk(new_xyz, "new_xyz", F32),
          _chk(idx, "idx", I32), _chk(w, "w", F32), int(w.shape[1]), _chk(dw, "dw", F32), int(dw.shape[1]),
          None if grad_new_xyz is None else _chk(grad_new_xyz, "grad_new_xyz", F32), _chk(scratch, "scratch", torch.uint8),
          b, n, m, ns, c1)
    return 1


def sa_point_gather(point_rows, xyz, new_xyz, idx, w, z, b, n, m, ns, c1, bias=None, relu=False):
    _numel_ok(point_rows, b * n * c1, "point_rows"); _numel_ok(z, b * m * ns * c1, "z"); _numel_ok(idx, b * m * ns, "idx")
    _numel_ok(xyz, b * n * 3, "xyz"); _numel_ok(new_xyz, b * m * 3, "new_xyz")
    assert w.shape[0] == c1 and w.shape[1] >= 3
    _call("pda_sa_point_gather", xyz, _chk(point_rows, "point_rows", F32), _chk(xyz, "xyz", F32), _chk(new_xyz, "new_xyz", F32),
          _chk(idx, "idx", I32), _chk(w, "w", F32), int(w.shape[1]), None if bias is None else _chk(bias, "bias", F32),
          1 if relu else 0, _chk(z, "z", F32), b, n, m, ns, c1)
    return 1
```

pdanet_amd/pointnet2_utils.py:

```python
from typing import List, Tuple

import os

import torch
import torch.nn as nn
from torch.autograd import Function

from . import _lib
from . import param_cache
from . import pointnet2_batch_cuda as pointnet2

_fwd = torch.amp.custom_fwd(device_type="cuda", cast_inputs=torch.float32)
_bwd = torch.amp.custom_bwd(device_type="cuda")


class FarthestPointSampling(Function):

    @staticmethod
    @_fwd
    def forward(ctx, xyz: torch.Tensor, npoint: int) -> torch.Tensor:
        assert xyz.is_contiguous()
        B, N, _ = xyz.size()
        output = torch.empty((B, npoint), dtype=torch.int32, device=xyz.device)
        temp = torch.full((B, N), 1e10, dtype=torch.float32, device=xyz.device)
# ... 960 lines not shown
        M, ns = idx.shape[1], idx.shape[2]
        C, n_out = feats_pm.shape[-1], weight.shape[0]
        xyz, new_xyz, feats_pm, idx = xyz.contiguous(), new_xyz.contiguous(), feats_pm.contiguous(), idx.contiguous()
        w = weight.detach().contiguous()
        w_f = w[:, 3:].contiguous()
        rows = _gemm_nt(feats_pm.view(B * N, C), w_f)
        z = torch.empty((B, M, ns, n_out), dtype=torch.float32, device=xyz.device)
        pointnet2.sa_point_gather(rows, xyz, new_xyz, idx, w, z, B, N, M, ns, n_out)
        ctx.save_for_backward(xyz, new_xyz, feats_pm, idx, weight)
        return z

    @staticmethod
    def backward(ctx, grad_out):
        xyz, new_xyz, feats_pm, idx, weight = ctx.saved_tensors
        B, M, ns = idx.shape
        n_out, C, N = weight.shape[0], feats_pm.shape[-1], xyz.shape[1]
        g2 = grad_out.contiguous().view(-1, n_out)
        g_new = g_feats = gw = None
        with torch.no_grad():
            w = weight.contiguous()
            if ctx.needs_input_grad[4] or ctx.needs_input_grad[1]:
                gw = torch.empty_like(weight)
                g_new = torch.empty_like(new_xyz) if ctx.needs_input_grad[1] else None
                pointnet2.sa_xyz_grad(g2, xyz, new_xyz, idx, w, gw, g_new, B, N, M, ns, n_out)
            if ctx.needs_input_grad[4] or ctx.needs_input_grad[2]:
                g_pts = torch.zeros((B, N, n_out), dtype=torch.float32, device=g2.device)
                pointnet2.group_rows_grad(B, N, n_out, M * ns, g2, idx, g_pts)
                g_pts = g_pts.view(B * N, n_out)
                if ctx.needs_input_grad[4]:
                    gw[:, 3:] = _wgrad(feats_pm.view(B * N, C), g_pts, torch.empty((n_out, C), dtype=weight.dtype, device=weight.device), False)[0]
                if ctx.needs_input_grad[2]:
                    g_feats = _gemm_nn(g_pts, w[:, 3:].contiguous()).view(B, N, C)
            if not ctx.needs_input_grad[4]:
                gw = None
        return None, g_new, g_feats, None, gw


SA_WIDE_INFER_SPLIT = os.environ.get("PDA_SA_WIDE_INFER_SPLIT", "1") != "0"
SA_WIDE_INFER_GATHER_IN_GEMM = os.environ.get("PDA_SA_WIDE_INFER_GATHER_IN_GEMM", "1") != "0"


def sa_wide_scale_infer(xyz, new_xyz, feats_pm, idx, folded):
    (w1, b1), (w2, b2), (w3, b3) = folded
    B, N, _ = xyz.shape
    M, ns = idx.shape[1], idx.shape[2]
    C = feats_pm.shape[-1]
    T = B * M * ns
    c1, c2, c3 = w1.shape[0], w2.shape[0], w3.shape[0]
    if not (SA_WIDE_INFER_SPLIT and SPLIT_GEMM and not DENSE_BF16 and w1.shape[1] == 3 + C and C % 32 == 0 and c1 in (128, 256, 512, 1024)
            and c1 % 32 == 0 and c2 % 128 == 0 and c3 % 128 == 0 and B * N >= SPLIT_GEMM_MIN_TOKENS and T >= SPLIT_GEMM_MIN_TOKENS):
        return None
    out = []

    def run():
        rows = _gemm_nt(feats_pm.reshape(B * N, C), w1[:, 3:].contiguous())
        if SA_WIDE_INFER_GATHER_IN_GEMM and c1 % 32 == 0 and c1 <= 1024:
            y2 = torch.empty((T, c2), dtype=torch.float32, device=xyz.device)
            pointnet2.gemm_split_gather(rows, xyz.contiguous(), new_xyz.contiguous(), idx.contiguous(), w1.contiguous(), b1.detach().contiguous(),
                                        _split_planes(w2), b2.detach().contiguous(), y2, B, N, M, ns, c1, c2, relu=True)
        else:
            y1 = torch.empty((T, c1), dtype=torch.float32, device=xyz.device)
            pointnet2.sa_point_gather(rows, xyz.contiguous(), new_xyz.contiguous(), idx.contiguous(), w1, y1, B, N, M, ns, c1, bias=b1, relu=True)
            y2 = _gemm_nt(y1, w2, b2, relu=True)
            del y1
        if ns in (16, 32, 64) and c2 % 32 == 0:
            pooled = torch.empty((B, M, c3), dtype=torch.float32, device=xyz.device)
            pointnet2.gemm_split_maxpool(y2, _split_planes(w3), b3.detach().contiguous(), pooled, T, c2, c3, ns, relu=True)
            out.append(pooled)
            return
        y3 = _gemm_nt(y2, w3, b3, relu=True)
        del y2
        out.append(y3.view(B, M, ns, c3).amax(dim=2))
    _sa_timed(2.0 * T * (c1 * c2 + c2 * c3), run, "bf16x6_infer")
    return out[0]


SA_SMALL_TRAIN = True
FUSED_WIDE_CHAIN_OK = True


class SaSmallChainTrain(Function):

    @staticmethod
    def supported(xyz, new_xyz, feats_pm, idx, mlp):
        layers = list(mlp)
        if not (SA_SMALL_TRAIN and len(layers) == 9 and xyz.is_cuda and xyz.dtype == torch.float32 and not DENSE_BF16
                and not torch.is_autocast_enabled() and not xyz.requires_grad and not new_xyz.requires_grad
                and (feats_pm is None or (feats_pm.dtype == torch.float32 and not feats_pm.requires_grad))):
            return False
        for k in range(3):
            conv, bn, act = layers[3 * k:3 * k + 3]
            if not (isinstance(conv, nn.Conv2d) and conv.bias is None and conv.kernel_size == (1, 1) and isinstance(bn, nn.BatchNorm2d)
                    and isinstance(act, nn.ReLU) and bn.training and bn.affine and bn.momentum is not None
                    and conv.weight.dtype == torch.float32):
                return False
        c = 0 if feats_pm is None else feats_pm.shape[-1]
        c1, c2, c3 = (layers[3 * k].out_channels for k in range(3))
        return layers[0].in_channels == 3 + c and pointnet2.sa_small_train_supported(c, idx.shape[2], c1, c2, c3, idx.numel())

    @staticmethod
    def forward(ctx, xyz, new_xyz, feats_pm, idx, w1, w2, w3, g1, b1, g2, b2, g3, b3, bns):
        B, N, _ = xyz.shape
        M, ns = idx.shape[1], idx.shape[2]
        c = 0 if feats_pm is None else feats_pm.shape[-1]
        c3 = w3.shape[0]
        dev = xyz.device
        xyz, new_xyz, idx = xyz.contiguous(), new_xyz.contiguous(), idx.contiguous()
        feats_pm = None if feats_pm is None else feats_pm.contiguous()
        ws = torch.empty((pointnet2.sa_small_train_workspace_bytes(),), dtype=torch.uint8, device=dev)
        out = torch.empty((B, M, c3), dtype=torch.float32, device=dev)
        zmax = torch.empty((B, M, c3), dtype=torch.float32, device=dev)
        arg = torch.empty((B, M, c3), dtype=torch.uint8, device=dev)
        track = [bn.track_running_stats for bn in bns]
        macs = w1.numel() + w2.numel() + w3.numel()
        _sa_timed(2.0 * B * M * ns * macs, lambda: pointnet2.sa_small_train_fwd(
            xyz, new_xyz, feats_pm, idx, (w1.contiguous(), w2.contiguous(), w3.contiguous()), (g1, g2, g3), (b1, b2, b3),
            [bn.running_mean if t else None for bn, t in zip(bns, track)],
            [bn.running_var if t else None for bn, t in zip(bns, track)],
            [bn.eps for bn in bns], [bn.momentum for bn in bns], ws, out, zmax, arg, B, N, M, c, ns), "f32_recompute")
        ctx.save_for_backward(xyz, new_xyz, feats_pm, idx, zmax, arg, ws, w1, w2, w3)
        ctx.dims = (B, N, M, c, ns)
        return out

    @staticmethod
    def backward(ctx, grad_out):
        xyz, new_xyz, feats_pm, idx, zmax, arg, ws, w1, w2, w3 = ctx.saved_tensors
        B, N, M, c, ns = ctx.dims
        tokens = B * M * ns
        dev = xyz.device
        dz2 = torch.empty((tokens, w2.shape[0]), dtype=torch.float32, device=dev)
        dz1 = torch.empty((tokens, w1.shape[0]), dtype=torch.float32, device=dev)
        dws = [torch.empty(w.shape, dtype=torch.float32, device=dev) for w in (w1, w2, w3)]
        dgs = [torch.empty((w.shape[0],), dtype=torch.float32, device=dev) for w in (w1, w2, w3)]
        dbs = [torch.empty((w.shape[0],), dtype=torch.float32, device=dev) for w in (w1, w2, w3)]
        gout = grad_out.contiguous().float()
        macs = w1.numel() + w2.numel() + w3.numel()
        _sa_timed(2.0 * tokens * (2 * macs - w1.numel()), lambda: pointnet2.sa_small_train_bwd(
            xyz, new_xyz, feats_pm, idx, gout, zmax, arg, ws, dz2, dz1, dws, dgs, dbs, B, N, M, c, ns), "f32_recompute")
        return (None, None, None, None, dws[0], dws[1], dws[2], dgs[0], dbs[0], dgs[1], dbs[1], dgs[2], dbs[2], None)


def sa_small_chain_train(xyz, new_xyz, feats_pm, idx, mlp):
    layers = list(mlp)
    convs, bns = [layers[0], layers[3], layers[6]], [layers[1], layers[4], layers[7]]
    for bn in bns:
        bump_bn_counter(bn)
    return SaSmallChainTrain.apply(xyz, new_xyz, feats_pm, idx, convs[0].weight.flatten(1), convs[1].weight.flatten(1),
                                   convs[2].weight.flatten(1), bns[0].weight, bns[0].bias, bns[1].weight, bns[1].bias,
                                   bns[2].weight, bns[2].bias, bns)


SA_WIDE_CHAIN = os.environ.get("PDA_SA_WIDE_CHAIN", "1") != "0"
WIDE_CHAIN_DGRAD_FIRST = os.environ.get("PDA_WIDE_CHAIN_DGRAD_FIRST", "1") != "0"
SA_WIDE_CHAIN_MIN_TOKENS = int(os.environ.get("PDA_SA_WIDE_CHAIN_MIN_TOKENS", "32768"))


class SaWideChainTrain(Function):

    @staticmethod
    def supported(xyz, new_xyz, feats_pm, idx, mlp):
        layers = list(mlp)
        if not (SA_WIDE_CHAIN and FUSED_WIDE_CHAIN_OK and len(layers) == 9 and feats_pm is not None and idx is not None):
            return False
        convs, bns = [layers[0], layers[3], layers[6]], [layers[1], layers[4], layers[7]]
        if not (all(isinstance(c, nn.Conv2d) and c.bias is None and c.weight.dtype == torch.float32 for c in convs)
                and all(isinstance(b, nn.BatchNorm2d) and b.affine and b.training and b.momentum is not None for b in bns)
                and all(isinstance(layers[k], nn.ReLU) for k in (2, 5, 8))):
            return False
        w1 = convs[0].weight.flatten(1)
        if not SaPointLinear.supported(xyz, feats_pm, w1):
            return False
        c1, c2, c3 = (c.weight.shape[0] for c in convs)
        T = idx.shape[0] * idx.shape[1] * idx.shape[2]
        if not (c1 % 256 == 0 and c2 % 256 == 0 and c3 % 256 == 0 and max(c1, c2, c3) <= 1024 and 1 <= idx.shape[2] <= 255
                and T >= SA_WIDE_CHAIN_MIN_TOKENS and not DENSE_BF16 and not torch.is_autocast_enabled()):
            return False
        lib = _lib.load()
        return int(lib.pda_linear_wgrad_form(T, c1, c2)) == 2 and int(lib.pda_linear_wgrad_form(T, c2, c3)) == 2

    @staticmethod
    def forward(ctx, xyz, new_xyz, feats_pm, idx, w1, w2, w3, g1, b1, g2, b2, g3, b3, bns):
        B, N, _ = xyz.shape
        M, ns = idx.shape[1], idx.shape[2]
        C, c1, c2, c3 = feats_pm.shape[-1], w1.shape[0], w2.shape[0], w3.shape[0]
        T = B * M * ns
        dev = xyz.device
        xyz, new_xyz, feats_pm, idx = xyz.contiguous(), new_xyz.contiguous(), feats_pm.contiguous(), idx.contiguous()
        gs = [t.detach().contiguous() for t in (g1, g2, g3)]
        bs = [t.detach().contiguous() for t in (b1, b2, b3)]
        stats = [(bn.running_mean, bn.running_var) if bn.track_running_stats else (None, None) for bn in bns]
        w1d = w1.detach().contiguous()
        rows = _gemm_nt(feats_pm.view(B * N, C), w1d[:, 3:].contiguous())
        z1 = torch.empty((T, c1), dtype=torch.float32, device=dev)
        pointnet2.sa_point_gather(rows, xyz, new_xyz, idx, w1d, z1, B, N, M, ns, c1)
        mi1 = torch.empty((2 * c1,), dtype=torch.float32, device=dev)
        scratch = torch.empty((pointnet2.bn_relu_scratch_bytes(c1),), dtype=torch.uint8, device=dev)
        pointnet2.bn_stats_fwd(z1, stats[0][0], stats[0][1], mi1, scratch, T, c1, bns[0].eps, bns[0].momentum)
        tiles = pointnet2.gemm_split_bn_tiles(T)

        def layer(z_in, mi_in, k, w, n_out, bn, st, gi, bi):
            z = torch.empty((T, n_out), dtype=torch.float32, device=dev)
            part = torch.empty((tiles * 2 * n_out,), dtype=torch.float64, device=dev)
            wf = _split_planes(w)
            _sa_timed(2.0 * T * k * n_out, lambda: pointnet2.gemm_split_bn(z_in, wf, z, T, k, n_out, in_bn=(mi_in, gi, bi), stats_mode=1,
                                                                           partial=part), "bf16x6")
            mi = torch.empty((2 * n_out,), dtype=torch.float32, device=dev)
            pointnet2.bn_finalize_fwd(part, tiles, n_out, T, bn.eps, bn.momentum, mi, st[0], st[1])
            return z, mi
        z2, mi2 = layer(z1, mi1, c1, w2, c2, bns[1], stats[1], gs[0], bs[0])
        z3, mi3 = layer(z2, mi2, c2, w3, c3, bns[2], stats[2], gs[1], bs[1])
        out = torch.empty((B, M, c3), dtype=torch.float32, device=dev)
        arg = torch.empty((B, M, c3), dtype=torch.uint8, device=dev)
        pointnet2.bn_relu_max_pool_apply(z3, gs[2], bs[2], mi3, out, arg, B * M, ns, c3)
        ctx.save_for_backward(xyz, new_xyz, feats_pm, idx, w1, w2, w3, g1, b1, g2, b2, g3, b3, z1, z2, z3, mi1, mi2, mi3, arg)
        return out

    @staticmethod
    def backward(ctx, grad_out):
        xyz, new_xyz, feats_pm, idx, w1, w2, w3, g1, b1, g2, b2, g3, b3, z1, z2, z3, mi1, mi2, mi3, arg = ctx.saved_tensors
        B, M, ns = idx.shape
        N, C = xyz.shape[1], feats_pm.shape[-1]
        c1, c2, c3 = w1.shape[0], w2.shape[0], w3.shape[0]
        T = B * M * ns
        dev = xyz.device
        tiles = pointnet2.gemm_split_bn_tiles(T)
        with torch.no_grad():
            g1c, b1c, g2c, b2c, g3c, b3c = (t.contiguous() for t in (g1, b1, g2, b2, g3, b3))
            gz3 = torch.empty((T, c3), dtype=torch.float32, device=dev)
            dg3, db3 = torch.empty_like(g3c), torch.empty_like(b3c)
            scratch = torch.empty((pointnet2.bn_relu_scratch_bytes(c3),), dtype=torch.uint8, device=dev)
            pointnet2.bn_relu_max_pool_bwd(z3, grad_out.contiguous().float(), arg, g3c, b3c, mi3, gz3, dg3, db3, scratch, B * M, ns, c3)

            def layer(gz, w, z_in, mi_in, gi, bi, k_in, n_out):
                dw = torch.empty((n_out, k_in), dtype=torch.float32, device=dev)
                ga = torch.empty((T, k_in), dtype=torch.float32, device=dev)
                if WIDE_CHAIN_DGRAD_FIRST:
                    _lin_cols(gz, w, ga, T, n_out, k_in, True)
                    pointnet2.linear_wgrad_bn(z_in, gz, dw, T, k_in, n_out, mi_in, gi, bi)
                else:
                    pointnet2.linear_wgrad_bn(z_in, gz, dw, T, k_in, n_out, mi_in, gi, bi)
                    _lin_cols(gz, w, ga, T, n_out, k_in, True)
                dg, db = torch.empty_like(gi), torch.empty_like(bi)
                scratch = torch.empty((pointnet2.bn_relu_scratch_bytes(k_in),), dtype=torch.uint8, device=dev)
                pointnet2.bn_relu_bwd(z_in, ga, gi, bi, mi_in, ga, dg, db, scratch, T, k_in)
                return dw, ga, dg, db
            dw3, gz2, dg2, db2 = layer(gz3, w3, z2, mi2, g2c, b2c, c2, c3)
            del gz3
            dw2, gz1, dg1, db1 = layer(gz2, w2, z1, mi1, g1c, b1c, c1, c2)
            del gz2
            w1c = w1.contiguous()
            dw1 = torch.empty_like(w1c)
            g_new = torch.empty_like(new_xyz) if ctx.needs_input_grad[1] else None
            pointnet2.sa_xyz_grad(gz1, xyz, new_xyz, idx, w1c, dw1, g_new, B, N, M, ns, c1)
            g_pts = torch.zeros((B, N, c1), dtype=torch.float32, device=dev)
            pointnet2.group_rows_grad(B, N, c1, M * ns, gz1, idx, g_pts)
            g_pts = g_pts.view(B * N, c1)
            dw1[:, 3:] = _wgrad(feats_pm.view(B * N, C), g_pts, torch.empty((c1, C), dtype=torch.float32, device=dev), False)[0]
            g_feats = _gemm_nn(g_pts, w1c[:, 3:].contiguous()).view(B, N, C) if ctx.needs_input_grad[2] else None
        return None, g_new, g_feats, None, dw1, dw2, dw3, dg1, db1, dg2, db2, dg3, db3, None


def sa_wide_chain_train(xyz, new_xyz, feats_pm, idx, mlp):
    layers = list(mlp)
    convs, bns = [layers[0], layers[3], layers[6]], [layers[1], layers[4], layers[7]]
    for bn in bns:
        bump_bn_counter(bn)
    return SaWideChainTrain.apply(xyz, new_xyz, feats_pm, idx, convs[0].weight.flatten(1), convs[1].weight.flatten(1),
                                  convs[2].weight.flatten(1), bns[0].weight, bns[0].bias, bns[1].weight, bns[1].bias,
                                  bns[2].weight, bns[2].bias, bns)


RAGGED_TOKENS = True
RAGGED_MAX_FRACTION = 0.85


class RaggedPlan:
    __slots__ = ("cnt", "off", "rowmap", "roww", "tokens", "groups", "nsample")

    def __init__(self, cnt, off, rowmap, roww, tokens, groups, nsample):
        self.cnt, self.off, self.rowmap, self.roww = cnt, off, rowmap, roww
        self.tokens, self.groups, self.nsample = tokens, groups, nsample

    @property
    def fraction(self):
        return self.tokens / float(self.groups * self.nsample)


def ragged_plan_parts(idxs):
    parts = []
    for idx in idxs:
        G, ns = idx.shape[0] * idx.shape[1], idx.shape[2]
        cnt = torch.empty((G,), dtype=torch.int32, device=idx.device)
        off = torch.empty((G + 1,), dtype=torch.int32, device=idx.device)
        rowmap = torch.empty((G * ns,), dtype=torch.int32, device=idx.device)
        roww = torch.empty((G * ns,), dtype=torch.float32, device=idx.device)
        pointnet2.ragged_plan(idx, cnt, off, rowmap, G, ns, roww)
        parts.append((cnt, off, rowmap, roww, G, ns))
    return parts, torch.stack([p[1][-1] for p in parts])


def ragged_plans_from(parts, totals):
    return [RaggedPlan(c, o, r[:u], w[:u], int(u), G, ns) for (c, o, r, w, G, ns), u in zip(parts, totals)]


def ragged_plans(idxs):
    parts, totals = ragged_plan_parts(idxs)
    return ragged_plans_from(parts, totals.tolist())


ASSEMBLE_BWD_TOKEN_PARALLEL = os.environ.get("PDA_ASSEMBLE_BWD_TOKEN_PARALLEL", "1") != "0"


class AssembleTokensRagged(Function):

    @staticmethod
    def forward(ctx, rppe, dscale, feats_pm, idx, glob, plan):
        B, M, ns = idx.shape
        C, N = feats_pm.shape[-1], feats_pm.shape[1]
        compact = rppe.dim() == 2
        rppe, dscale, feats_pm, glob = rppe.contiguous(), dscale.contiguous(), feats_pm.contiguous(), glob.contiguous()
        out = torch.empty((plan.tokens, 4 * C), dtype=torch.float32, device=rppe.device)
        pointnet2.assemble_tokens_ragged(rppe, dscale, feats_pm, idx, glob, plan.rowmap, plan.off, out, plan.tokens, B, N, M, ns, C,
                                         rppe_compact=compact)
        ctx.save_for_backward(dscale, feats_pm, idx, plan.cnt, plan.off, plan.rowmap)
        ctx.dims = (B, N, M, ns, C, plan.tokens, compact)
        return out

    @staticmethod
    def backward(ctx, grad_out):
        dscale, feats_pm, idx, cnt, off, rowmap = ctx.saved_tensors
        B, N, M, ns, C, U, compact = ctx.dims
        dev = grad_out.device
        g_rppe = torch.empty((U, C) if compact else (B, M, ns, C), dtype=torch.float32, device=dev)
        g_ds = torch.empty_like(dscale)
        g_feats = torch.zeros((B, N, C), dtype=torch.float32, device=dev)
        g_glob = torch.empty((B, M, C), dtype=torch.float32, device=dev)
        pointnet2.assemble_tokens_ragged_grad(grad_out.contiguous(), dscale, feats_pm, idx, cnt, off, g_rppe, g_ds, g_feats, g_glob,
                                              U, B, N, M, ns, C, rppe_compact=compact,
                                              rowmap=rowmap if ASSEMBLE_BWD_TOKEN_PARALLEL else None)
        return g_rppe, g_ds, g_feats, None, g_glob, None


RAGGED_POSITION_MLP = True


class BatchNormReLUWeighted(Function):

    @staticmethod
    def forward(ctx, x, weight, bias, running_mean, running_var, eps, momentum, roww, count):
        x = x.contiguous()
        rows, c = x.shape
        y = torch.empty_like(x)
        stats = torch.empty((2 * c,), dtype=torch.float32, device=x.device)
        scratch = torch.empty((pointnet2.bn_relu_scratch_bytes(c),), dtype=torch.uint8, device=x.device)
        pointnet2.bn_relu_fwd_weighted(x, weight, bias, running_mean, running_var, y, stats, scratch, rows, c, eps, momentum, roww, count)
        ctx.save_for_backward(x, weight, bias, stats, roww)
        ctx.count = count
        return y

    @staticmethod
    def backward(ctx, grad_y):
        x, weight, bias, stats, roww = ctx.saved_tensors
        rows, c = x.shape
        gx = torch.empty_like(x)
        gw, gb = torch.empty_like(weight), torch.empty_like(bias)
        scratch = torch.empty((pointnet2.bn_relu_scratch_bytes(c),), dtype=torch.uint8, device=x.device)
        pointnet2.bn_relu_bwd_weighted(x, grad_y.contiguous(), weight, bias, stats, gx, gw, gb, scratch, rows, c, roww, ctx.count)
        return gx, gw, gb, None, None, None, None, None, None


def position_mlp_ragged_supported(layers, rppe):
    layers = list(layers)
    ok = (RAGGED_POSITION_MLP and rppe.is_cuda and rppe.dtype == torch.float32 and len(layers) == 6 and torch.is_grad_enabled()
          and not DENSE_BF16 and not torch.is_autocast_enabled())
    if not ok:
        return False
    for conv, bn in ((layers[0], layers[1]), (layers[3], layers[4])):
        c = conv.weight.shape[0]
        if (conv.bias is not None or not bn.training or not bn.affine or bn.momentum is None or c < 4 or c > 1024
                or (c & (c - 1)) != 0):
            return False
    return True


def position_mlp_ragged(layers, rppe, plan):
    layers = list(layers)
    x = rppe.reshape(-1, rppe.shape[-1]).index_select(0, plan.rowmap)
    count = plan.groups * plan.nsample
    for conv, bn in ((layers[0], layers[1]), (layers[3], layers[4])):
        x = linear(x, conv.weight.flatten(1), None)
        rm, rv = (bn.running_mean, bn.running_var) if bn.track_running_stats else (None, None)
        bump_bn_counter(bn)
        x = BatchNormReLUWeighted.apply(x, bn.weight, bn.bias, rm, rv, bn.eps, bn.momentum, plan.roww, count)
    return x


def _wgrad_ragged(x2d, g2d, weight, want_bias):
    n_out, n_in = weight.shape
    tokens = x2d.shape[0]
    if (LINEAR_WGRAD_KERNEL and tokens >= 4096 and (min(n_out, n_in) >= 64 or max(n_out, n_in) <= 64) and n_out % 4 == 0
            and n_in % 4 == 0 and x2d.dtype == torch.float32 and g2d.dtype == torch.float32):
        gw = torch.empty_like(weight)
        gb = torch.empty((n_out,), dtype=torch.float32, device=x2d.device) if want_bias else None
        pointnet2.linear_wgrad(x2d.contiguous(), g2d.contiguous(), gw, gb, tokens, n_in, n_out)
        return gw, gb
    return g2d.t().mm(x2d), (g2d.sum(0) if want_bias else None)


# ... 308 lines not shown
```

Measured before the change: 121.4 scenes/s.

## Fuse BN stats into SA point gather and BN backward into point grad

In the wide SA chain, the first-layer gather now also accumulates per-block double-precision BN sums, which replaces a separate stats pass over z1. In backward, the first BN's grad-x apply is folded into a new kernel that recomputes the BN/ReLU gradient on the fly and produces dW xyz columns, grad_new_xyz and the scatter into point rows in one pass. This replaces the separate sa_xyz_grad, group_rows_grad and bn_relu_bwd passes and avoids re-reading and re-writing the large T×c1 tensor. The cost is more register pressure and serialized per-group atomics in the fused kernel.

Measured after the change: 124.2 scenes/s (median of 6 runs). +2.3%, better.

```diff
diff --git a/include/pda_train.h b/include/pda_train.h
--- a/include/pda_train.h
+++ b/include/pda_train.h
@@ -18,6 +18,9 @@
 int pda_bn_relu_bwd(const float *x, const float *grad_y, const float *gamma, const float *beta,
                     const float *mean_invstd, float *grad_x, float *grad_gamma, float *grad_beta,
                     void *scratch, int64_t rows, int c, pda_stream_t stream);
+int pda_bn_relu_bwd_reduce(const float *x, const float *grad_y, const float *gamma, const float *beta,
+                           const float *mean_invstd, float *grad_gamma, float *grad_beta, float *sums, void *scratch,
+                           int64_t rows, int c, pda_stream_t stream);
 int pda_bn_relu_fwd_mixed(const void *x, int x_is_bf16, const float *gamma, const float *beta, float *running_mean,
                           float *running_var, void *y, int y_is_bf16, float *mean_invstd, void *scratch,
                           int64_t rows, int c, float eps, float momentum, pda_stream_t stream);
@@ -225,6 +228,14 @@
 int pda_sa_xyz_grad(const float *grad_z1, const float *xyz, const float *new_xyz, const int32_t *idx, const float *w, int ldw,
                     float *dw, int lddw, float *grad_new_xyz, void *scratch, int b, int n, int m, int nsample, int c1,
                     pda_stream_t stream);
+int64_t pda_sa_point_gather_stats_blocks(int64_t tokens, int c1);
+int pda_sa_point_gather_stats(const float *point_rows, const float *xyz, const float *new_xyz, const int32_t *idx,
+                              const float *w, int ldw, float *z, double *partial, int b, int n, int m, int nsample, int c1,
+                              pda_stream_t stream);
+int pda_sa_point_grad_bn(const float *grad_a1, const float *z1, const float *mean_invstd, const float *gamma,
+                         const float *beta, const float *bwd_sums, const float *xyz, const float *new_xyz, const int32_t *idx,
+                         const float *w, int ldw, float *dw, int lddw, float *grad_new_xyz, float *grad_points, void *scratch,
+                         int b, int n, int m, int nsample, int c1, pda_stream_t stream);
 
 int64_t pda_input_stage_workspace_bytes(int batch, int64_t n_cap);
 int pda_input_stage(const float *points, const int64_t *offsets, int64_t n_total, int batch, int c, int64_t n_cap,
diff --git a/pdanet_amd/_lib.py b/pdanet_amd/_lib.py
--- a/pdanet_amd/_lib.py
+++ b/pdanet_amd/_lib.py
@@ -100,6 +100,7 @@
     "pda_bn_stats_fwd": [_vp, _vp, _vp, _vp, _vp, ctypes.c_int64, _i, _f, _f, _vp],
     "pda_bn_finalize_fwd": [_vp, _i, _i, ctypes.c_int64, _f, _f, _vp, _vp, _vp, _vp],
     "pda_bn_relu_max_pool_apply": [_vp, _vp, _vp, _vp, _vp, _vp, ctypes.c_int64, _i, _i, _vp],
+    "pda_bn_relu_bwd_reduce": [_vp, _vp, _vp, _vp, _vp, _vp, _vp, _vp, _vp, ctypes.c_int64, _i, _vp],
     "pda_colsum_scratch_bytes": [_i],
     "pda_colsum_bf16": [_vp, _vp, _vp, ctypes.c_int64, _i, _vp],
     "pda_assemble_tokens": [_vp, _vp, _vp, _vp, _vp, _vp, _i, _i, _i, _i, _i, _vp],
@@ -153,6 +154,9 @@
     "pda_sa_xyz_grad_scratch_bytes": [_i],
     "pda_sa_point_gather": [_vp, _vp, _vp, _vp, _vp, _i, _vp, _i, _vp, _i, _i, _i, _i, _i, _vp],
     "pda_sa_xyz_grad": [_vp, _vp, _vp, _vp, _vp, _i, _vp, _i, _vp, _vp, _i, _i, _i, _i, _i, _vp],
+    "pda_sa_point_gather_stats_blocks": [ctypes.c_int64, _i],
+    "pda_sa_point_gather_stats": [_vp, _vp, _vp, _vp, _vp, _i, _vp, _vp, _i, _i, _i, _i, _i, _vp],
+    "pda_sa_point_grad_bn": [_vp] * 10 + [_i, _vp, _i, _vp, _vp, _vp, _i, _i, _i, _i, _i, _vp],
     "pda_adam_onecycle_step": [_vp, _vp, _vp, _vp, ctypes.c_int64, _f, _f, _f, _f, _f, _i, _vp, _f, _vp],
     "pda_input_stage_workspace_bytes": [_i, ctypes.c_int64],
     "pda_input_stage": [_vp, _vp, ctypes.c_int64, _i, _i, ctypes.c_int64, ctypes.POINTER(_f), _i, _vp, _vp, _vp,
@@ -262,7 +266,8 @@
     "pda_nms_mask_words", "pda_ball_query_cells_scratch_bytes", "pda_bn_relu_scratch_bytes",
     "pda_layer_norm_scratch_bytes", "pda_linear_wgrad_scratch_bytes", "pda_linear_split_packed_bytes",
     "pda_colsum_scratch_bytes", "pda_gemm_split_bn_tiles", "pda_densitynet_scratch_bytes",
-    "pda_sa_small_train_workspace_bytes", "pda_sa_xyz_grad_scratch_bytes", "pda_input_stage_workspace_bytes",
+    "pda_sa_small_train_workspace_bytes", "pda_sa_xyz_grad_scratch_bytes", "pda_sa_point_gather_stats_blocks",
+    "pda_input_stage_workspace_bytes",
     "pda_augment_workspace_bytes", "pda_augment_steps_workspace_bytes", "pda_once_eval_workspace_bytes",
     "pda_kitti_eval_workspace_bytes", "pda_kitti_fov_filter_workspace_bytes", "pda_gt_extract_workspace_bytes",
     "pda_voxel_workspace_bytes", "pda_dyn_voxel_workspace_bytes", "pda_center_focal_blocks", "pda_anchor_loss_blocks",
diff --git a/pdanet_amd/csrc/bn_relu.hip b/pdanet_amd/csrc/bn_relu.hip
--- a/pdanet_amd/csrc/bn_relu.hip
+++ b/pdanet_amd/csrc/bn_relu.hip
@@ -351,6 +351,24 @@
                                                  (hipStream_t)stream, "pda_bn_relu_bwd");
 }
 
+PDA_API int pda_bn_relu_bwd_reduce(const float* x, const float* grad_y, const float* gamma, const float* beta, const float* mean_invstd,
+                                   float* grad_gamma, float* grad_beta, float* sums, void* scratch, int64_t rows, int c,
+                                   pda_stream_t stream) {
+    const char* what = "pda_bn_relu_bwd_reduce";
+    pda::BnShape s;
+    if (int rc = pda::bn_shape(rows, c, s, what)) return rc;
+    PDA_REQUIRE(x && grad_y && gamma && beta && mean_invstd && grad_gamma && grad_beta && sums && scratch, "%s: null pointer", what);
+    PDA_REQUIRE(pda::bn_aligned(x) && pda::bn_aligned(grad_y) && (((uintptr_t)gamma | (uintptr_t)beta | (uintptr_t)mean_invstd) & 15) == 0,
+                "%s: pointers must be 16-byte aligned", what);
+    const int grid = pda::bn_grid(s);
+    hipStream_t st = (hipStream_t)stream;
+    hipLaunchKernelGGL((pda::bn_reduce_kernel<true, float, float>), dim3(grid), dim3(256), 0, st, x, grad_y, mean_invstd, gamma, beta,
+                       (double*)scratch, s);
+    hipLaunchKernelGGL(pda::bn_finalize_bwd_kernel, dim3(pda::divup(c, 32)), dim3(512), 0, st, (const double*)scratch, grid, c, s.count,
+                       grad_gamma, grad_beta, sums);
+    return pda::check_launch(what);
+}
+
 PDA_API int pda_bn_relu_fwd_weighted(const float* x, const float* gamma, const float* beta, float* running_mean, float* running_var,
                                      float* y, float* mean_invstd, void* scratch, int64_t rows, int c, float eps, float momentum,
                                      const float* row_weight, int64_t count, pda_stream_t stream) {
diff --git a/pdanet_amd/csrc/sa_xyz_grad.hip b/pdanet_amd/csrc/sa_xyz_grad.hip
--- a/pdanet_amd/csrc/sa_xyz_grad.hip
+++ b/pdanet_amd/csrc/sa_xyz_grad.hip
@@ -98,11 +98,12 @@
     }
 }
 
+template <bool STATS>
 __global__ __launch_bounds__(256) void sa_point_gather_kernel(const float* __restrict__ prow, const float* __restrict__ xyz,
                                                               const float* __restrict__ new_xyz, const int32_t* __restrict__ idx,
                                                               const float* __restrict__ w, int ldw, const float* __restrict__ bias,
                                                               int relu, float* __restrict__ z, int n, int m, int ns, int c1,
-                                                              int64_t tokens) {
+                                                              int64_t tokens, double* __restrict__ partial) {
     const int cq = c1 >> 2;
     const int q = threadIdx.x % cq;
     float wx[4], wy[4], wz[4];
@@ -114,6 +115,7 @@
     float bq[4] = {0.f, 0.f, 0.f, 0.f};
     if (bias) { const float4 b4 = *reinterpret_cast<const float4*>(bias + 4 * q); bq[0] = b4.x; bq[1] = b4.y; bq[2] = b4.z; bq[3] = b4.w; }
     const int tpb = 256 / cq;
+    double s1[4] = {0, 0, 0, 0}, s2[4] = {0, 0, 0, 0};
     for (int64_t tok = (int64_t)blockIdx.x * tpb + threadIdx.x / cq; tok < tokens; tok += (int64_t)gridDim.x * tpb) {
         const int64_t grp = tok / ns;
         const int bs = (int)(grp / m);
@@ -130,31 +132,233 @@
             o[k] = relu ? fmaxf(o[k], 0.f) : o[k];
         }
         *reinterpret_cast<float4*>(z + tok * c1 + 4 * q) = make_float4(o[0], o[1], o[2], o[3]);
-    }
-}
-
-}
-
-PDA_API int pda_sa_point_gather(const float* point_rows, const float* xyz, const float* new_xyz, const int32_t* idx, const float* w, int ldw,
-                                const float* bias, int relu, float* z, int b, int n, int m, int ns, int c1, pda_stream_t stream) {
-    using namespace pda;
-    PDA_REQUIRE(b >= 0 && n >= 1 && m >= 0 && ns >= 1 && c1 >= 4 && (c1 & 3) == 0 && ldw >= 3, "pda_sa_point_gather: bad size");
+        if constexpr (STATS) {
+#pragma unroll
+            for (int k = 0; k < 4; ++k) { s1[k] += (double)o[k]; s2[k] += (double)o[k] * (double)o[k]; }
+        }
+    }
+    if constexpr (STATS) {
+        __shared__ double lds[2 * 256 * 4];
+        double* la = lds;
+        double* lb = lds + 256 * 4;
+        const int tid = threadIdx.x;
+#pragma unroll
+        for (int k = 0; k < 4; ++k) { la[tid * 4 + k] = s1[k]; lb[tid * 4 + k] = s2[k]; }
+        __syncthreads();
+        if (tid < cq) {
+            double a[4] = {0, 0, 0, 0}, b[4] = {0, 0, 0, 0};
+            for (int r = 0; r < tpb; ++r)
+#pragma unroll
+                for (int k = 0; k < 4; ++k) { a[k] += la[(r * cq + tid) * 4 + k]; b[k] += lb[(r * cq + tid) * 4 + k]; }
+            double* pa = partial + (size_t)blockIdx.x * 2 * c1;
+#pragma unroll
+            for (int k = 0; k < 4; ++k) { pa[4 * tid + k] = a[k]; pa[c1 + 4 * tid + k] = b[k]; }
+        }
+    }
+}
+
+constexpr int PG_BLOCKS = 512;
+
+template <int CPT>
+__global__ __launch_bounds__(XG_THREADS) void sa_point_grad_bn_kernel(const float* __restrict__ ga, const float* __restrict__ z,
+                                                                      const float* __restrict__ mean_invstd, const float* __restrict__ gamma,
+                                                                      const float* __restrict__ beta, const float* __restrict__ sums,
+                                                                      const float* __restrict__ xyz, const float* __restrict__ new_xyz,
+                                                                      const int32_t* __restrict__ idx, const float* __restrict__ w, int ldw,
+                                                                      float* __restrict__ partial, float* __restrict__ grad_new,
+                                                                      float* __restrict__ g_pts, int n, int m, int ns, int c1, int64_t groups) {
+    __shared__ float red[XG_THREADS / 64][3];
+    const int tid = threadIdx.x;
+    float accw[CPT][3], wx[CPT][3], mu[CPT], is[CPT], gm[CPT], be[CPT], m1[CPT], m2[CPT];
+#pragma unroll
+    for (int q = 0; q < CPT; ++q) {
+        const int o = tid + q * XG_THREADS;
+        const bool ok = o < c1;
+#pragma unroll
+        for (int d = 0; d < 3; ++d) { accw[q][d] = 0.f; wx[q][d] = ok ? w[(size_t)o * ldw + d] : 0.f; }
+        mu[q] = ok ? mean_invstd[o] : 0.f; is[q] = ok ? mean_invstd[c1 + o] : 0.f;
+        gm[q] = ok ? gamma[o] : 0.f; be[q] = ok ? beta[o] : 0.f;
+        m1[q] = ok ? sums[o] : 0.f; m2[q] = ok ? sums[c1 + o] : 0.f;
+    }
+    for (int64_t grp = blockIdx.x; grp < groups; grp += gridDim.x) {
+        const int bs = (int)(grp / m);
+        const float* ct = new_xyz + grp * 3;
+        const float cx = ct[0], cy = ct[1], cz = ct[2];
+        const float* pts = xyz + (size_t)bs * n * 3;
+        const int32_t* ids = idx + grp * ns;
+        const float* grow = ga + grp * ns * (int64_t)c1;
+        const float* zrow = z + grp * ns * (int64_t)c1;
+        float* prow = g_pts + (size_t)bs * n * c1;
+        float gs[CPT], run[CPT];
+#pragma unroll
+        for (int q = 0; q < CPT; ++q) { gs[q] = 0.f; run[q] = 0.f; }
+        int run_id = -1;
+        auto flush = [&]() {
+            if ((unsigned)run_id < (unsigned)n) {
+#pragma unroll
+                for (int q = 0; q < CPT; ++q) {
+                    const int o = tid + q * XG_THREADS;
+                    if (o < c1) atomicAdd(prow + (size_t)run_id * c1 + o, run[q]);
+                }
+            }
+        };
+        for (int s0 = 0; s0 < ns; s0 += 8) {
+            float gv[8][CPT], zv[8][CPT], dx[8], dy[8], dz[8];
+            int id[8];
+#pragma unroll
+            for (int u = 0; u < 8; ++u) {
+                const int s = s0 + u < ns ? s0 + u : ns - 1;
+                id[u] = ids[s];
+                const float* pt = pts + (size_t)id[u] * 3;
+                dx[u] = pt[0] - cx; dy[u] = pt[1] - cy; dz[u] = pt[2] - cz;
+#pragma unroll
+                for (int q = 0; q < CPT; ++q) {
+                    const int o = tid + q * XG_THREADS;
+                    const bool ok = s0 + u < ns && o < c1;
+                    gv[u][q] = ok ? grow[(int64_t)s * c1 + o] : 0.f;
+                    zv[u][q] = ok ? zrow[(int64_t)s * c1 + o] : 0.f;
+                }
+            }
+#pragma unroll
+            for (int u = 0; u < 8; ++u) {
+                const bool live = s0 + u < ns;
+                float gz[CPT];
+#pragma unroll
+                for (int q = 0; q < CPT; ++q) {
+                    const int o = tid + q * XG_THREADS;
+                    const float wgt = 1.f;
+                    const float xh = (zv[u][q] - mu[q]) * is[q];
+                    const float dyh = (xh * gm[q] + be[q] > 0.f) ? gv[u][q] : 0.f;
+                    const float v = gm[q] * is[q] * (dyh - wgt * (m1[q] + xh * m2[q]));
+                    gz[q] = (live && o < c1) ? v : 0.f;
+                    accw[q][0] = __builtin_fmaf(gz[q], dx[u], accw[q][0]);
+                    accw[q][1] = __builtin_fmaf(gz[q], dy[u], accw[q][1]);
+                    accw[q][2] = __builtin_fmaf(gz[q], dz[u], accw[q][2]);
+                    gs[q] += gz[q];
+                }
+                if (live) {
+                    if (id[u] == run_id) {
+#pragma unroll
+                        for (int q = 0; q < CPT; ++q) run[q] += gz[q];
+                    } else {
+                        flush();
+                        run_id = id[u];
+#pragma unroll
+                        for (int q = 0; q < CPT; ++q) run[q] = gz[q];
+                    }
+                }
+            }
+        }
+        flush();
+        if (grad_new) {
+            float v[3] = {0.f, 0.f, 0.f};
+#pragma unroll
+            for (int q = 0; q < CPT; ++q)
+#pragma unroll
+                for (int d = 0; d < 3; ++d) v[d] = __builtin_fmaf(gs[q], wx[q][d], v[d]);
+#pragma unroll
+            for (int d = 0; d < 3; ++d) {
+#pragma unroll
+                for (int o = 32; o >= 1; o >>= 1) v[d] += __shfl_xor(v[d], o);
+            }
+            __syncthreads();
+            if (lane_id() == 0) { red[wave_id()][0] = v[0]; red[wave_id()][1] = v[1]; red[wave_id()][2] = v[2]; }
+            __syncthreads();
+            if (tid < 3) grad_new[grp * 3 + tid] = -((red[0][tid] + red[1][tid]) + (red[2][tid] + red[3][tid]));
+        }
+    }
+#pragma unroll
+    for (int q = 0; q < CPT; ++q) {
+        const int o = tid + q * XG_THREADS;
+        if (o < c1) {
+            float* p = partial + ((size_t)blockIdx.x * c1 + o) * 3;
+            p[0] = accw[q][0]; p[1] = accw[q][1]; p[2] = accw[q][2];
+        }
+    }
+}
+
+constexpr int PG_STATS_BLOCKS = 1024;
+
+static int gather_blocks(int64_t tokens, int c1, int cap) {
+    const int64_t steps = divup64(tokens * (c1 >> 2), 256);
+    return (int)(steps < cap ? steps : cap);
+}
+
+static int launch_point_gather(const float* point_rows, const float* xyz, const float* new_xyz, const int32_t* idx, const float* w, int ldw,
+                               const float* bias, int relu, float* z, double* partial, bool stats, int b, int n, int m, int ns, int c1,
+                               hipStream_t stream, const char* what) {
+    PDA_REQUIRE(b >= 0 && n >= 1 && m >= 0 && ns >= 1 && c1 >= 4 && (c1 & 3) == 0 && ldw >= 3, "%s: bad size", what);
     const int64_t tokens = (int64_t)b * m * ns;
     if (tokens == 0) return PDA_OK;
     PDA_REQUIRE(point_rows && xyz && new_xyz && idx && w && z && (((uintptr_t)point_rows | (uintptr_t)z | (uintptr_t)bias) & 15) == 0,
-                "pda_sa_point_gather: null or misaligned pointer");
+                "%s: null or misaligned pointer", what);
+    PDA_REQUIRE(!stats || (partial && ((uintptr_t)partial & 7) == 0), "%s: null or misaligned partial", what);
     if (256 % (c1 >> 2) != 0) {
-        set_error("pda_sa_point_gather: c1 = %d (c1 / 4 must divide 256)", c1);
+        set_error("%s: c1 = %d (c1 / 4 must divide 256)", what, c1);
         return PDA_ERR_UNSUPPORTED;
     }
-    const int64_t total = tokens * (c1 >> 2);
-    const int blocks = (int)(divup64(total, 256) < 8192 ? divup64(total, 256) : 8192);
-    hipLaunchKernelGGL(sa_point_gather_kernel, dim3(blocks), dim3(256), 0, (hipStream_t)stream, point_rows, xyz, new_xyz, idx, w, ldw, bias, relu, z,
-                       n, m, ns, c1, tokens);
-    return check_launch("pda_sa_point_gather");
-}
-
-PDA_API int64_t pda_sa_xyz_grad_scratch_bytes(int c1) { return c1 > 0 ? (int64_t)pda::XG_BLOCKS * c1 * 3 * sizeof(float) : 0; }
+    if (stats)
+        hipLaunchKernelGGL(sa_point_gather_kernel<true>, dim3(gather_blocks(tokens, c1, PG_STATS_BLOCKS)), dim3(256), 0, stream, point_rows, xyz,
+                           new_xyz, idx, w, ldw, bias, relu, z, n, m, ns, c1, tokens, partial);
+    else
+        hipLaunchKernelGGL(sa_point_gather_kernel<false>, dim3(gather_blocks(tokens, c1, 8192)), dim3(256), 0, stream, point_rows, xyz, new_xyz,
+                           idx, w, ldw, bias, relu, z, n, m, ns, c1, tokens, (double*)nullptr);
+    return check_launch(what);
+}
+
+}
+
+PDA_API int pda_sa_point_gather(const float* point_rows, const float* xyz, const float* new_xyz, const int32_t* idx, const float* w, int ldw,
+                                const float* bias, int relu, float* z, int b, int n, int m, int ns, int c1, pda_stream_t stream) {
+    return pda::launch_point_gather(point_rows, xyz, new_xyz, idx, w, ldw, bias, relu, z, nullptr, false, b, n, m, ns, c1, (hipStream_t)stream,
+                                    "pda_sa_point_gather");
+}
+
+PDA_API int64_t pda_sa_point_gather_stats_blocks(int64_t tokens, int c1) {
+    return tokens > 0 && c1 >= 4 ? pda::gather_blocks(tokens, c1, pda::PG_STATS_BLOCKS) : 0;
+}
+
+PDA_API int pda_sa_point_gather_stats(const float* point_rows, const float* xyz, const float* new_xyz, const int32_t* idx, const float* w,
+                                      int ldw, float* z, double* partial, int b, int n, int m, int ns, int c1, pda_stream_t stream) {
+    return pda::launch_point_gather(point_rows, xyz, new_xyz, idx, w, ldw, nullptr, 0, z, partial, true, b, n, m, ns, c1, (hipStream_t)stream,
+                                    "pda_sa_point_gather_stats");
+}
+
+PDA_API int64_t pda_sa_xyz_grad_scratch_bytes(int c1) {
+    constexpr int blocks = pda::XG_BLOCKS > pda::PG_BLOCKS ? pda::XG_BLOCKS : pda::PG_BLOCKS;
+    return c1 > 0 ? (int64_t)blocks * c1 * 3 * sizeof(float) : 0;
+}
+
+PDA_API int pda_sa_point_grad_bn(const float* grad_a1, const float* z1, const float* mean_invstd, const float* gamma, const float* beta,
+                                 const float* bwd_sums, const float* xyz, const float* new_xyz, const int32_t* idx, const float* w, int ldw,
+                                 float* dw, int lddw, float* grad_new_xyz, float* grad_points, void* scratch, int b, int n, int m, int ns,
+                                 int c1, pda_stream_t stream) {
+    using namespace pda;
+    PDA_REQUIRE(b >= 0 && n >= 1 && m >= 0 && ns >= 1 && c1 >= 1 && ldw >= 3 && lddw >= 3, "pda_sa_point_grad_bn: bad size");
+    PDA_REQUIRE(grad_points || (int64_t)b * c1 == 0, "pda_sa_point_grad_bn: null pointer");
+    const hipStream_t s = (hipStream_t)stream;
+    if ((int64_t)b * c1 > 0) {
+        const hipError_t e = hipMemsetAsync(grad_points, 0, (size_t)b * n * c1 * sizeof(float), s);
+        PDA_REQUIRE(e == hipSuccess, "pda_sa_point_grad_bn: hipMemsetAsync: %s", hipGetErrorString(e));
+    }
+    const int64_t groups = (int64_t)b * m;
+    if (groups == 0) return PDA_OK;
+    PDA_REQUIRE(grad_a1 && z1 && mean_invstd && gamma && beta && bwd_sums && xyz && new_xyz && idx && w && dw && scratch,
+                "pda_sa_point_grad_bn: null pointer");
+    if (c1 > XG_THREADS * XG_MAXC) {
+        set_error("pda_sa_point_grad_bn: c1 = %d > %d", c1, XG_THREADS * XG_MAXC);
+        return PDA_ERR_UNSUPPORTED;
+    }
+    const int blocks = (int)(groups < PG_BLOCKS ? groups : PG_BLOCKS);
+    float* partial = (float*)scratch;
+    const int cpt = divup(c1, XG_THREADS);
+#define PDA_PG(CPT) hipLaunchKernelGGL((sa_point_grad_bn_kernel<CPT>), dim3(blocks), dim3(XG_THREADS), 0, s, grad_a1, z1, mean_invstd, gamma, beta, \
+                                       bwd_sums, xyz, new_xyz, idx, w, ldw, partial, grad_new_xyz, grad_points, n, m, ns, c1, groups)
+    if (cpt == 1) PDA_PG(1); else if (cpt == 2) PDA_PG(2); else PDA_PG(4);
+#undef PDA_PG
+    hipLaunchKernelGGL(sa_xyz_grad_reduce_kernel, dim3(divup(c1 * 3, 16)), dim3(256), 0, s, (const float*)partial, blocks, c1, dw, lddw);
+    return check_launch("pda_sa_point_grad_bn");
+}
 
 PDA_API int pda_sa_xyz_grad(const float* grad_z1, const float* xyz, const float* new_xyz, const int32_t* idx, const float* w, int ldw,
                             float* dw, int lddw, float* grad_new_xyz, void* scratch, int b, int n, int m, int ns, int c1,
diff --git a/pdanet_amd/pointnet2_batch_cuda.py b/pdanet_amd/pointnet2_batch_cuda.py
--- a/pdanet_amd/pointnet2_batch_cuda.py
+++ b/pdanet_amd/pointnet2_batch_cuda.py
@@ -289,6 +289,15 @@
     _call("pda_bn_relu_bwd_mixed", x, xp, xb, gp, gb, _chk(gamma, "gamma", F32), _chk(beta, "beta", F32),
           _chk(mean_invstd, "mean_invstd", F32), _chk(grad_x, "grad_x", x.dtype), _chk(grad_gamma, "grad_gamma", F32),
           _chk(grad_beta, "grad_beta", F32), _chk(scratch, "scratch", torch.uint8), rows, c)
+    return 1
+
+
+def bn_relu_bwd_reduce(x, grad_y, gamma, beta, mean_invstd, grad_gamma, grad_beta, sums, scratch, rows, c):
+    _numel_ok(x, rows * c, "x"); _numel_ok(grad_y, rows * c, "grad_y"); _numel_ok(sums, 2 * c, "sums")
+    _numel_ok(grad_gamma, c, "grad_gamma"); _numel_ok(grad_beta, c, "grad_beta"); _numel_ok(mean_invstd, 2 * c, "mean_invstd")
+    _call("pda_bn_relu_bwd_reduce", x, _chk(x, "x", F32), _chk(grad_y, "grad_y", F32), _chk(gamma, "gamma", F32), _chk(beta, "beta", F32),
+          _chk(mean_invstd, "mean_invstd", F32), _chk(grad_gamma, "grad_gamma", F32), _chk(grad_beta, "grad_beta", F32),
+          _chk(sums, "sums", F32), _chk(scratch, "scratch", torch.uint8), rows, c)
     return 1
 
 
@@ -825,3 +834,36 @@
           _chk(idx, "idx", I32), _chk(w, "w", F32), int(w.shape[1]), None if bias is None else _chk(bias, "bias", F32),
           1 if relu else 0, _chk(z, "z", F32), b, n, m, ns, c1)
     return 1
+
+
+@functools.lru_cache(maxsize=None)
+def sa_point_gather_stats_blocks(tokens, c1):
+    return int(_lib.load().pda_sa_point_gather_stats_blocks(int(tokens), int(c1)))
+
+
+def sa_point_gather_stats(point_rows, xyz, new_xyz, idx, w, z, partial, b, n, m, ns, c1):
+    _numel_ok(point_rows, b * n * c1, "point_rows"); _numel_ok(z, b * m * ns * c1, "z"); _numel_ok(idx, b * m * ns, "idx")
+    _numel_ok(xyz, b * n * 3, "xyz"); _numel_ok(new_xyz, b * m * 3, "new_xyz")
+    _numel_ok(partial, sa_point_gather_stats_blocks(b * m * ns, c1) * 2 * c1, "partial")
+    assert w.shape[0] == c1 and w.shape[1] >= 3
+    _call("pda_sa_point_gather_stats", xyz, _chk(point_rows, "point_rows", F32), _chk(xyz, "xyz", F32), _chk(new_xyz, "new_xyz", F32),
+          _chk(idx, "idx", I32), _chk(w, "w", F32), int(w.shape[1]), _chk(z, "z", F32), _chk(partial, "partial", torch.float64),
+          b, n, m, ns, c1)
+    return 1
+
+
+def sa_point_grad_bn(grad_a1, z1, mean_invstd, gamma, beta, bwd_sums, xyz, new_xyz, idx, w, dw, grad_new_xyz, grad_points, b, n, m, ns, c1):
+    t = b * m * ns
+    _numel_ok(grad_a1, t * c1, "grad_a1"); _numel_ok(z1, t * c1, "z1"); _numel_ok(idx, t, "idx")
+    _numel_ok(mean_invstd, 2 * c1, "mean_invstd"); _numel_ok(gamma, c1, "gamma"); _numel_ok(beta, c1, "beta"); _numel_ok(bwd_sums, 2 * c1, "bwd_sums")
+    _numel_ok(xyz, b * n * 3, "xyz"); _numel_ok(new_xyz, b * m * 3, "new_xyz"); _numel_ok(grad_points, b * n * c1, "grad_points")
+    if grad_new_xyz is not None:
+        _numel_ok(grad_new_xyz, b * m * 3, "grad_new_xyz")
+    assert w.shape[0] == c1 and dw.shape == w.shape and w.shape[1] >= 3
+    scratch = torch.empty((sa_xyz_grad_scratch_bytes(c1),), dtype=torch.uint8, device=xyz.device)
+    _call("pda_sa_point_grad_bn", xyz, _chk(grad_a1, "grad_a1", F32), _chk(z1, "z1", F32), _chk(mean_invstd, "mean_invstd", F32),
+          _chk(gamma, "gamma", F32), _chk(beta, "beta", F32), _chk(bwd_sums, "bwd_sums", F32), _chk(xyz, "xyz", F32),
+          _chk(new_xyz, "new_xyz", F32), _chk(idx, "idx", I32), _chk(w, "w", F32), int(w.shape[1]), _chk(dw, "dw", F32), int(dw.shape[1]),
+          None if grad_new_xyz is None else _chk(grad_new_xyz, "grad_new_xyz", F32), _chk(grad_points, "grad_points", F32),
+          _chk(scratch, "scratch", torch.uint8), b, n, m, ns, c1)
+    return 1
diff --git a/pdanet_amd/pointnet2_utils.py b/pdanet_amd/pointnet2_utils.py
--- a/pdanet_amd/pointnet2_utils.py
+++ b/pdanet_amd/pointnet2_utils.py
@@ -1136,6 +1136,7 @@
 
 SA_WIDE_CHAIN = os.environ.get("PDA_SA_WIDE_CHAIN", "1") != "0"
 WIDE_CHAIN_DGRAD_FIRST = os.environ.get("PDA_WIDE_CHAIN_DGRAD_FIRST", "1") != "0"
+SA_WIDE_FUSED_ENDS = os.environ.get("PDA_SA_WIDE_FUSED_ENDS", "1") != "0"
 SA_WIDE_CHAIN_MIN_TOKENS = int(os.environ.get("PDA_SA_WIDE_CHAIN_MIN_TOKENS", "32768"))
 
 
@@ -1176,10 +1177,16 @@
         w1d = w1.detach().contiguous()
         rows = _gemm_nt(feats_pm.view(B * N, C), w1d[:, 3:].contiguous())
         z1 = torch.empty((T, c1), dtype=torch.float32, device=dev)
-        pointnet2.sa_point_gather(rows, xyz, new_xyz, idx, w1d, z1, B, N, M, ns, c1)
         mi1 = torch.empty((2 * c1,), dtype=torch.float32, device=dev)
-        scratch = torch.empty((pointnet2.bn_relu_scratch_bytes(c1),), dtype=torch.uint8, device=dev)
-        pointnet2.bn_stats_fwd(z1, stats[0][0], stats[0][1], mi1, scratch, T, c1, bns[0].eps, bns[0].momentum)
+        if SA_WIDE_FUSED_ENDS:
+            nb1 = pointnet2.sa_point_gather_stats_blocks(T, c1)
+            part1 = torch.empty((nb1 * 2 * c1,), dtype=torch.float64, device=dev)
+            pointnet2.sa_point_gather_stats(rows, xyz, new_xyz, idx, w1d, z1, part1, B, N, M, ns, c1)
+            pointnet2.bn_finalize_fwd(part1, nb1, c1, T, bns[0].eps, bns[0].momentum, mi1, stats[0][0], stats[0][1])
+        else:
+            pointnet2.sa_point_gather(rows, xyz, new_xyz, idx, w1d, z1, B, N, M, ns, c1)
+            scratch = torch.empty((pointnet2.bn_relu_scratch_bytes(c1),), dtype=torch.uint8, device=dev)
+            pointnet2.bn_stats_fwd(z1, stats[0][0], stats[0][1], mi1, scratch, T, c1, bns[0].eps, bns[0].momentum)
         tiles = pointnet2.gemm_split_bn_tiles(T)
 
         def layer(z_in, mi_in, k, w, n_out, bn, st, gi, bi):
@@ -1215,7 +1222,7 @@
             scratch = torch.empty((pointnet2.bn_relu_scratch_bytes(c3),), dtype=torch.uint8, device=dev)
             pointnet2.bn_relu_max_pool_bwd(z3, grad_out.contiguous().float(), arg, g3c, b3c, mi3, gz3, dg3, db3, scratch, B * M, ns, c3)
 
-            def layer(gz, w, z_in, mi_in, gi, bi, k_in, n_out):
+            def layer(gz, w, z_in, mi_in, gi, bi, k_in, n_out, sums=None):
                 dw = torch.empty((n_out, k_in), dtype=torch.float32, device=dev)
                 ga = torch.empty((T, k_in), dtype=torch.float32, device=dev)
                 if WIDE_CHAIN_DGRAD_FIRST:
@@ -1226,18 +1233,26 @@
                     _lin_cols(gz, w, ga, T, n_out, k_in, True)
                 dg, db = torch.empty_like(gi), torch.empty_like(bi)
                 scratch = torch.empty((pointnet2.bn_relu_scratch_bytes(k_in),), dtype=torch.uint8, device=dev)
-                pointnet2.bn_relu_bwd(z_in, ga, gi, bi, mi_in, ga, dg, db, scratch, T, k_in)
+                if sums is not None:
+                    pointnet2.bn_relu_bwd_reduce(z_in, ga, gi, bi, mi_in, dg, db, sums, scratch, T, k_in)
+                else:
+                    pointnet2.bn_relu_bwd(z_in, ga, gi, bi, mi_in, ga, dg, db, scratch, T, k_in)
                 return dw, ga, dg, db
             dw3, gz2, dg2, db2 = layer(gz3, w3, z2, mi2, g2c, b2c, c2, c3)
             del gz3
-            dw2, gz1, dg1, db1 = layer(gz2, w2, z1, mi1, g1c, b1c, c1, c2)
+            sums1 = torch.empty((2 * c1,), dtype=torch.float32, device=dev) if SA_WIDE_FUSED_ENDS else None
+            dw2, gz1, dg1, db1 = layer(gz2, w2, z1, mi1, g1c, b1c, c1, c2, sums1)
             del gz2
             w1c = w1.contiguous()
             dw1 = torch.empty_like(w1c)
             g_new = torch.empty_like(new_xyz) if ctx.needs_input_grad[1] else None
-            pointnet2.sa_xyz_grad(gz1, xyz, new_xyz, idx, w1c, dw1, g_new, B, N, M, ns, c1)
-            g_pts = torch.zeros((B, N, c1), dtype=torch.float32, device=dev)
-            pointnet2.group_rows_grad(B, N, c1, M * ns, gz1, idx, g_pts)
+            if SA_WIDE_FUSED_ENDS:
+                g_pts = torch.empty((B, N, c1), dtype=torch.float32, device=dev)
+                pointnet2.sa_point_grad_bn(gz1, z1, mi1, g1c, b1c, sums1, xyz, new_xyz, idx, w1c, dw1, g_new, g_pts, B, N, M, ns, c1)
+            else:
+                pointnet2.sa_xyz_grad(gz1, xyz, new_xyz, idx, w1c, dw1, g_new, B, N, M, ns, c1)
+                g_pts = torch.zeros((B, N, c1), dtype=torch.float32, device=dev)
+                pointnet2.group_rows_grad(B, N, c1, M * ns, gz1, idx, g_pts)
             g_pts = g_pts.view(B * N, c1)
             dw1[:, 3:] = _wgrad(feats_pm.view(B * N, C), g_pts, torch.empty((c1, C), dtype=torch.float32, device=dev), False)[0]
             g_feats = _gemm_nn(g_pts, w1c[:, 3:].contiguous()).view(B, N, C) if ctx.needs_input_grad[2] else None
```
